# lRomul/sensorium

Measured on AMD Instinct MI355X. Metric: training clips/sec/GPU (DwiseNeuro fwd+bwd, B=32 T=32 36x64) at 1/2/4/8 GPUs, higher is better.
Workload: dtype bf16

## Files before the change

sensorium_amd/_lib.py:

```python
from __future__ import annotations

import ctypes as C
import os
from pathlib import Path

import torch

_HERE = Path(__file__).resolve().parent
DETERMINISTIC = os.environ.get("DWN_DETERMINISTIC", "0") == "1"
_LIB_NAME = "libdwiseneuro_hip_det.so" if DETERMINISTIC else "libdwiseneuro_hip.so"
LIB_PATH = Path(os.environ["DWN_LIB_PATH"]) if os.environ.get("DWN_LIB_PATH") else _HERE / "csrc" / _LIB_NAME

c_p = C.c_void_p
c_i = C.c_int
c_ll = C.c_longlong
c_f = C.c_float
c_d = C.c_double
c_sz = C.c_size_t

DWN_F32, DWN_BF16 = 0, 1
DWN_NREP = 32
LD_PLAIN, LD_PE, LD_BNACT, LD_AFFINE2, LD_DY3, LD_GATE, LD_CAT1 = 0, 1, 2, 3, 4, 5, 6
EPI_STORE, EPI_READOUT, EPI_DG, EPI_STORE_CAT, EPI_DH3 = 0, 1, 2, 3, 4
NN_AUTO, NN_XL128, NN_XL256, NN_TILE128, NN_KD = 0, 1, 2, 3, 4
# ... 248 lines not shown
    _fields_ = [("N", c_i), ("L", c_i), ("gh", c_i), ("gw", c_i), ("fit_baseline", c_i), ("pad_", c_i), ("params", c_p), ("maps", c_p),
                ("profile", c_p), ("separability", c_p)]


CORR_STAT_ROWS, CORR_TILE = 8, 16
CORR_MEAN, CORR_SUM = 0, 1
GABOR_GAUSSIAN, GABOR_NONE = 0, 1
BLUR_MAX_RADIUS, BLUR_TAPS_STRIDE, MOMENTS_CHUNK = 16, 33, 4096
MEI_STEP, MEI_PROJECT = 0, 1
MEI_CONTRAST_MAX, MEI_CONTRAST_FIXED = 0, 1
TRIAL_STATE_ROWS, TRIAL_SCORE_ROWS, TRIAL_SUMMARY, TRIAL_TILE = 17, 5, 8, 4
NOISE_BINARY, NOISE_SPARSE = 0, 1
STA_SUMMARY = 8
GAUSS_PARAMS, GAUSS_TABLE = 7, 16
PAIR_TOTAL, PAIR_SIGNAL, PAIR_NOISE = 0, 1, 2
PAIR_TILE, PAIR_KSTEP, PAIR_SUMMARY, PAIR_ROW_STATS = 64, 4, 8, 8
MIX_BOX, MIX_BLEND = 0, 1
VID_U8, VID_F32 = 0, 1

_OLD_STRUCTS = {
    "dwn_load_desc": LoadDesc, "dwn_gemm_nn_args": GemmNNArgs, "dwn_gemm_tn_args": GemmTNArgs,
    "dwn_dw_spatial_fwd_args": DwSpatialFwdArgs, "dwn_dw_spatial_bwd_args": DwSpatialBwdArgs,
    "dwn_dw_temporal_fwd_args": DwTemporalFwdArgs, "dwn_dw_temporal_bwd_args": DwTemporalBwdArgs,
    "dwn_bn": BN, "dwn_stem_args": StemArgs, "dwn_block_args": BlockArgs, "dwn_pool_args": PoolArgs,
    "dwn_cortex_args": CortexArgs, "dwn_readout_args": ReadoutArgs, "dwn_tensor_entry": TensorEntry,
    "dwn_clip_src": ClipSrc, "dwn_clip_desc": ClipDesc, "dwn_pw_bwd_args": PwBwdArgs,
    "dwn_dw_spatial_rc_fwd_args": DwSpatialRcFwdArgs,
}
_NEW_STRUCTS = {
    "dwn_stem_input_grad_args": StemInputGradArgs,
    "dwn_guarded_entry": GuardedEntry, "dwn_step_guard": StepGuard, "dwn_gaze_args": GazeArgs,
    "dwn_corr_args": CorrArgs, "dwn_gabor_args": GaborArgs, "dwn_modulator_args": ModulatorArgs,
    "dwn_blur3d_args": Blur3dArgs, "dwn_clip_moments_args": ClipMomentsArgs, "dwn_mei_update_args": MeiUpdateArgs,
    "dwn_trial_desc": TrialDesc, "dwn_trial_group": TrialGroup, "dwn_trial_score_args": TrialScoreArgs,
    "dwn_spatial_gain_args": SpatialGainArgs, "dwn_noise_args": NoiseArgs, "dwn_sta_args": StaArgs,
    "dwn_gauss2d_args": Gauss2dArgs, "dwn_gauss2d_profile_args": Gauss2dProfileArgs,
    "dwn_pair_seg": PairSeg, "dwn_pair_args": PairArgs, "dwn_pair_compare_args": PairCompareArgs,
}
_STRUCTS = {**_OLD_STRUCTS, **_NEW_STRUCTS}


class _new(tuple):
    def __new__(cls, restype, argtypes):
        return super().__new__(cls, (restype, argtypes))


_P = C.POINTER
SYMBOLS = {
    "dwn_abi_version": (c_i, []),
    "dwn_source_hash": (C.c_char_p, []),
    "dwn_sizeof": (c_i, [C.c_char_p]),
    "dwn_last_error": (C.c_char_p, []),
    "dwn_profile_enable": (c_i, [C.c_ulonglong, c_i]),
    "dwn_profile_collect": (c_i, [c_i, _P(c_d), _P(c_ll)]),
    "dwn_gemm_nn": (c_i, [_P(GemmNNArgs), c_i, c_i, c_p]),
    "dwn_gemm_tn": (c_i, [_P(GemmTNArgs), c_i, c_i, c_p]),
    "dwn_dw_spatial_fwd": (c_i, [_P(DwSpatialFwdArgs), c_i, c_i, c_p]),
    "dwn_dw_spatial_bwd": (c_i, [_P(DwSpatialBwdArgs), c_i, c_i, c_p]),
    "dwn_dw_spatial_bwd_rc_supported": (c_i, [_P(DwSpatialBwdArgs), c_i]),
    "dwn_dw_spatial_fwd_rc_supported": (c_i, [_P(DwSpatialFwdArgs), c_i]),
    "dwn_dw_temporal_fwd": (c_i, [_P(DwTemporalFwdArgs), c_i, c_i, c_p]),
    "dwn_dw_temporal_bwd": (c_i, [_P(DwTemporalBwdArgs), c_i, c_i, c_p]),
    "dwn_dw_temporal_wide_fwd": _new(c_i, [_P(DwTemporalFwdArgs), c_i, c_i, c_p]),
    "dwn_dw_temporal_wide_bwd": _new(c_i, [_P(DwTemporalBwdArgs), c_i, c_i, c_p]),
    "dwn_bn_finalize": (c_i, [c_p, c_i, c_d, _P(BN), c_i, c_i, c_f, c_f, c_i, c_p]),
    "dwn_bn_bwd_finalize": (c_i, [c_p, c_d, _P(BN), c_p, c_i, c_i, c_p]),
    "dwn_pack_weight": (c_i, [c_p, c_p, c_i, c_i, c_i, c_i, c_i, c_i, c_i, c_i, c_p]),
    "dwn_stem_workspace_bytes": (c_sz, [_P(StemArgs)]),
    "dwn_stem_forward": (c_i, [_P(StemArgs), c_i, c_p]),
    "dwn_stem_backward": (c_i, [_P(StemArgs), c_i, c_p]),
    "dwn_stem_input_grad": _new(c_i, [_P(StemInputGradArgs), c_i, c_p]),
    "dwn_stem_backward_input": _new(c_i, [_P(StemArgs), c_p, c_i, c_p]),
    "dwn_block_workspace_bytes": (c_sz, [_P(BlockArgs), c_i]),
    "dwn_block_forward": (c_i, [_P(BlockArgs), c_i, c_p]),
    "dwn_block_backward": (c_i, [_P(BlockArgs), c_i, c_p]),
    "dwn_block_forward_writes": (c_i, [_P(BlockArgs)]),
    "dwn_pool_forward": (c_i, [_P(PoolArgs), c_i, c_p]),
    "dwn_pool_backward": (c_i, [_P(PoolArgs), c_i, c_p]),
    "dwn_cortex_workspace_bytes": (c_sz, [_P(CortexArgs), c_i]),
    "dwn_cortex_forward": (c_i, [_P(CortexArgs), c_i, c_p]),
    "dwn_cortex_backward": (c_i, [_P(CortexArgs), c_i, c_p]),
    "dwn_readout_workspace_bytes": (c_sz, [_P(ReadoutArgs), c_i]),
    "dwn_readout_wt_bytes": (c_sz, [_P(ReadoutArgs)]),
    "dwn_readout_forward": (c_i, [_P(ReadoutArgs), c_i, c_p]),
    "dwn_readout_backward": (c_i, [_P(ReadoutArgs), c_i, c_p]),
    "dwn_poisson_loss_forward": (c_i, [c_p, c_p, c_p, c_ll, c_ll, c_f, c_p, c_i, c_p]),
    "dwn_poisson_loss_backward": (c_i, [c_p, c_p, c_p, c_p, c_ll, c_ll, c_f, c_p, c_i, c_p]),
    "dwn_f64_to_f32": (c_i, [c_p, c_p, c_i, c_i, c_p]),
    "dwn_adamw_ema_multi": (c_i, [c_p, c_i, c_i, c_d, c_d, c_d, c_d, c_d, c_ll, c_d, c_d, c_i, c_p]),
    "dwn_ema_lerp_multi": (c_i, [c_p, c_i, c_i, c_d, c_i, c_p]),
    "dwn_grad_guard_workspace_bytes": _new(c_sz, [c_i, c_i]),
    "dwn_grad_sumsq_multi": _new(c_i, [c_p, c_i, c_i, c_d, c_p, c_sz, c_p, c_i, c_p]),
    "dwn_step_guard_finalize": _new(c_i, [c_p, c_p, c_d, c_i, c_p, c_i, c_p, c_i, c_p]),
    "dwn_adamw_ema_multi_guarded": _new(c_i, [c_p, c_i, c_i, c_d, c_d, c_d, c_d, c_d, c_d, c_d, c_p, c_i, c_p]),
    "dwn_conv_pw_bn_stats_workspace_bytes": (c_sz, [c_i]),
    "dwn_conv_pw_bn_stats": (c_i, [c_p, c_ll, c_ll, c_p, c_i, c_i, _P(BN), c_f, c_f, c_p, c_p, c_sz, c_i, c_i, c_p]),
    "dwn_pw_bwd_fused_supported": (c_i, [c_i, c_ll, c_i, c_i]),
    "dwn_pw_backward_workspace_bytes": (c_sz, [c_i, c_i, c_i]),
    "dwn_pw_backward": (c_i, [_P(PwBwdArgs), c_i, c_i, c_p]),
    "dwn_dw_spatial_rc_blob_bytes": (c_sz, [c_i, c_i]),
    "dwn_dw_spatial_rc_prep": (c_i, [c_p, c_p, c_p, c_i, c_i, c_p, c_i, c_p]),
    "dwn_dw_spatial_rc_supported": (c_i, [c_i, c_i, c_i, c_i, c_i, c_i, c_i]),
    "dwn_dw_spatial_fwd_rc": (c_i, [_P(DwSpatialRcFwdArgs), c_i, c_p]),
    "dwn_assemble_inputs": (c_i, [c_p, c_i, c_i, c_i, c_i, c_i, c_i, c_f, c_p, c_i, c_p]),
    "dwn_assemble_targets": (c_i, [c_p, c_i, c_i, c_p, c_p, c_i, c_i, c_p, c_i, c_p]),
    "dwn_gaze_shift_forward": _new(c_i, [_P(GazeArgs), c_i, c_p]),
    "dwn_gaze_shift_backward": _new(c_i, [_P(GazeArgs), c_i, c_p]),
    "dwn_plane_mean": _new(c_i, [c_p, c_i, c_i, c_i, c_i, c_i, c_i, c_i, c_p, c_i, c_p]),
    "dwn_corr_ws_bytes": _new(c_sz, [_P(CorrArgs)]),
    "dwn_corr_moments": _new(c_i, [_P(CorrArgs), c_i, c_p]),
    "dwn_corr_loss_finalize": _new(c_i, [_P(CorrArgs), c_i, c_p]),
    "dwn_corr_loss_backward": _new(c_i, [_P(CorrArgs), c_i, c_p]),
    "dwn_gabor_workspace_bytes": _new(c_sz, [_P(GaborArgs)]),
    "dwn_gabor_forward": _new(c_i, [_P(GaborArgs), c_i, c_p]),
    "dwn_gabor_backward": _new(c_i, [_P(GaborArgs), c_i, c_p]),
    "dwn_modulator_ws_bytes": _new(c_sz, [_P(ModulatorArgs)]),
    "dwn_modulator_forward": _new(c_i, [_P(ModulatorArgs), c_i, c_p]),
    "dwn_modulator_backward": _new(c_i, [_P(ModulatorArgs), c_i, c_p]),
    "dwn_blur3d_ws_bytes": _new(c_sz, [_P(Blur3dArgs)]),
    "dwn_clip_moments_ws_bytes": _new(c_sz, [_P(ClipMomentsArgs)]),
    "dwn_blur3d": _new(c_i, [_P(Blur3dArgs), c_i, c_p]),
    "dwn_clip_moments": _new(c_i, [_P(ClipMomentsArgs), c_i, c_p]),
    "dwn_mei_update": _new(c_i, [_P(MeiUpdateArgs), c_i, c_p]),
    "dwn_trial_score_ws_bytes": _new(c_sz, [_P(TrialScoreArgs)]),
    "dwn_trial_moments": _new(c_i, [_P(TrialScoreArgs), c_i, c_p]),
    "dwn_trial_score_finalize": _new(c_i, [_P(TrialScoreArgs), c_i, c_p]),
    "dwn_spatial_gain_ws_bytes": _new(c_sz, [_P(SpatialGainArgs)]),
    "dwn_spatial_gain_forward": _new(c_i, [_P(SpatialGainArgs), c_i, c_p]),
    "dwn_spatial_gain_backward": _new(c_i, [_P(SpatialGainArgs), c_i, c_p]),
    "dwn_pair_ldz": _new(c_ll, [c_i]),
    "dwn_pair_state_bytes": _new(c_sz, [_P(PairArgs)]),
    "dwn_pair_ws_bytes": _new(c_sz, [_P(PairArgs)]),
    "dwn_pair_compare_ws_bytes": _new(c_sz, [_P(PairCompareArgs)]),
    "dwn_pair_stage": _new(c_i, [_P(PairArgs), c_i, c_p]),
    "dwn_pair_syrk": _new(c_i, [_P(PairArgs), c_i, c_p]),
    "dwn_pair_corr_finalize": _new(c_i, [_P(PairArgs), c_i, c_p]),
    "dwn_pair_compare": _new(c_i, [_P(PairCompareArgs), c_i, c_p]),
    "dwn_gauss2d_ws_bytes": _new(c_sz, [_P(Gauss2dArgs)]),
    "dwn_gauss2d_fit": _new(c_i, [_P(Gauss2dArgs), c_i, c_p]),
    "dwn_gauss2d_profile": _new(c_i, [_P(Gauss2dProfileArgs), c_i, c_p]),
    "dwn_noise_forward": _new(c_i, [_P(NoiseArgs), c_i, c_p]),
    "dwn_sta_state_bytes": _new(c_sz, [_P(StaArgs)]),
    "dwn_sta_ws_bytes": _new(c_sz, [_P(StaArgs)]),
    "dwn_sta_accumulate": _new(c_i, [_P(StaArgs), c_i, c_p]),
    "dwn_sta_finalize": _new(c_i, [_P(StaArgs), c_i, c_p]),
}


class DwnError(RuntimeError):
    pass


HASH_SRCS = ("dwn_api.hip", "dwn_gemm.hip", "dwn_gemm_nn_1.hip", "dwn_gemm_nn_2.hip", "dwn_gemm_nn_3.hip", "dwn_gemm_nn_4.hip", "dwn_gemm_nn_5.hip",
             "dwn_gemm_nn_6.hip", "dwn_gemm_tn.hip", "dwn_pw_bwd.hip", "dwn_gemm_xl.hip", "dwn_gemm_kd.hip", "dwn_dwconv.hip", "dwn_dwrc.hip",
             "dwn_dwbwd.hip", "dwn_dwfwd.hip", "dwn_elementwise.hip", "dwn_data.hip", "dwn_gaze.hip", "dwn_modulator.hip", "dwn_spatial.hip", "dwn_mei.hip", "dwn_rf_fit.hip", "dwn_pairwise.hip", "dwn_trial_score.hip", "dwn_rf.hip", "dwn_corr.hip", "dwn_stim.hip", "dwn_common.h", "dwn_internal.h",
             "dwn_kernels.h", "dwn_launch.h", "dwn_gemm_nn.h", "dwn_gain.h", "dwn_reduce.h",
             "../../include/dwn.h")


def source_hash() -> str:
    import hashlib
    h = hashlib.sha256()
    for name in HASH_SRCS:
        h.update((_HERE / "csrc" / name).read_bytes())
    return h.hexdigest()[:16]


def _load():
    if not LIB_PATH.exists():
        raise ImportError(
            f"{LIB_PATH} is missing: build it with `python -c 'import __graft_entry__ as g; g.build()'` "
            f"(or `make -C {LIB_PATH.parent}`).  sensorium_amd has no fallback path.")
    lib = C.CDLL(str(LIB_PATH), mode=getattr(os, "RTLD_NOW", 2))
    ab = bool(os.environ.get("DWN_LIB_PATH"))
    for name, proto in SYMBOLS.items():
        if ab and isinstance(proto, _new) and not hasattr(lib, name):
            continue
        restype, argtypes = proto
        fn = getattr(lib, name)
        fn.restype = restype
        fn.argtypes = argtypes
    if lib.dwn_abi_version() != 7 and not (ab and lib.dwn_abi_version() == 6):
        raise ImportError("libdwiseneuro_hip.so ABI version mismatch")
    built, have = lib.dwn_source_hash().decode(), source_hash()
    if built != have and not os.environ.get("DWN_LIB_PATH"):
        raise ImportError(f"{LIB_PATH.name} was built from other sources (binary {built}, tree {have}): rebuild it with "
                          f"`make -C {LIB_PATH.parent}` — binaries are not in git, so what runs must be what is committed")
    for cname, struct in _STRUCTS.items():
        n = lib.dwn_sizeof(cname.encode())
        if n != C.sizeof(struct) and not (ab and (0 < n < C.sizeof(struct) or cname in _NEW_STRUCTS)):
            raise ImportError(f"struct layout mismatch for {cname}: C {n} bytes vs ctypes {C.sizeof(struct)}")
    return lib


lib = _load()


def check(rc: int, what: str = ""):
    if rc != 0:
        msg = lib.dwn_last_error()
        raise DwnError(f"{what} failed (rc={rc}): {msg.decode() if msg else ''}")
```

sensorium_amd/csrc/dwn_api.hip:

```cpp
#include "dwn_internal.h"
#include "dwn_kernels.h"
#include <string.h>
#include <math.h>

static thread_local char g_err[512] = "";
#ifndef DWN_EVAL_CHAIN
#define DWN_EVAL_CHAIN 1
#endif

extern "C" size_t dwn_dw_spatial_rc_blob_bytes(int E, int Cin);
extern "C" int dwn_dw_spatial_rc_supported(int dtype, int Cin, int E, int ks, int stride, int Hin, int Win);
extern "C" int dwn_dw_spatial_rc_prep(const float* w_pw, const float* w_dws, const float* bn1_coef, int E, int Cin, void* blob,
                                      int device, void* stream);
extern "C" int dwn_dw_spatial_fwd_rc(const dwn_dw_spatial_rc_fwd_args* a, int device, void* stream);
bool dw_spatial_bwd_rc_supported(const DwSpatialBwd& a, int dtype);
bool dw_spatial_fwd_rc_walk_supported(const DwSpatialFwd& a, int dtype);

int dwn_set_error(int code, const char* msg) {
    snprintf(g_err, sizeof(g_err), "dwn error %d: %s", code, msg ? msg : "");
    return code;
}

#define TRY(x) do { int rc__ = (x); if (rc__ != 0) return rc__; } while (0)

// ... 45 lines not shown
        }
        if (range) g_roctx_pop();
    }
};
}
#define PROF(fam, call) do { ProfScope ps__((fam), s); TRY(call); } while (0)
#define HIP_TRY(x) do { hipError_t e__ = (x); if (e__ != hipSuccess) return dwn_set_error((int)e__, hipGetErrorString(e__)); } while (0)
#define ENTER(device) do { g_err[0] = 0; HIP_TRY(hipSetDevice(device)); } while (0)

namespace {

struct Carver {
    char* base; size_t off; size_t cap;
    explicit Carver(void* b, size_t c) : base((char*)b), off(0), cap(c) {}
    template <class U> U* take(size_t n) {
        off = (off + 255) & ~(size_t)255;
        U* p = base ? (U*)(base + off) : (U*)nullptr;
        off += n * sizeof(U);
        return p;
    }
    bool ok() const { return base == nullptr || off <= cap; }
};

inline size_t tsize(int dtype) { return dtype == DWN_BF16 ? 2 : 4; }
inline size_t nstat(int C) { return (size_t)DWN_NREP * 2 * C; }

LoadDesc ld_plain(const void* p, i64 ld) {
    LoadDesc d; memset(&d, 0, sizeof(d));
    d.p = p; d.ld = ld;
    return d;
}
LoadDesc ld_bnact(const void* p, i64 ld, const float* coef, int C, int act, const float* gate, int gate_ld,
                  int rows_per_sample) {
    LoadDesc d = ld_plain(p, ld);
    d.v1 = coef; d.v2 = coef + C; d.act = act; d.gate = gate; d.gate_ld = gate_ld;
    d.rows_per_sample = rows_per_sample > 0 ? rows_per_sample : 1;
    return d;
}
LoadDesc ld_affine2(const void* p, const void* q, i64 ld, const float* abc, int C) {
    LoadDesc d = ld_plain(p, ld);
    d.q = q; d.v1 = abc; d.v2 = abc + C; d.v3 = abc + 2 * C;
    return d;
}
LoadDesc ld_pe(const void* p, i64 ld, const float* pe_t, const float* pe_h, const float* pe_w, int T, int H, int W) {
    LoadDesc d = ld_plain(p, ld);
    d.pe_t = pe_t; d.pe_h = pe_h; d.pe_w = pe_w; d.pT = T; d.pH = H; d.pW = W; d.pe_ld = (int)ld;
    return d;
}
LoadDesc ld_ycoef(const void* y, i64 ld, const float* coef, int C) {
    LoadDesc d = ld_plain(y, ld);
    d.v1 = coef; d.v2 = coef + C; d.v3 = coef + 2 * C; d.v4 = coef + 3 * C;
    return d;
}

BnFinJob fin_job(const double* stats, int stat_c, double count, const dwn_bn& bn, int C) {
    BnFinJob j; memset(&j, 0, sizeof(j));
    j.stats = stats; j.stat_c = stat_c; j.count = count; j.gamma = bn.gamma; j.beta = bn.beta;
    j.running_mean = bn.running_mean; j.running_var = bn.running_var; j.nbt = bn.num_batches_tracked; j.coef = bn.coef; j.C = C;
    return j;
}
BnBwdJob bwd_job(const double* stats, double count, const dwn_bn& bn, float* abc, int C, bool frozen) {
    BnBwdJob j; memset(&j, 0, sizeof(j));
    j.stats = stats; j.count = count; j.coef = bn.coef; j.dgamma = bn.dgamma; j.dbeta = bn.dbeta; j.abc = abc; j.C = C;
    j.frozen = frozen ? 1 : 0;
    return j;
}

int bn_finalize(const double* stats, int stat_c, double count, const dwn_bn& bn, int C, int training, float momentum,
                float eps, hipStream_t s) {
    if (training) return k_bn_finalize_train(fin_job(stats, stat_c, count, bn, C), BnFinJob{}, momentum, eps, s);
    return k_bn_finalize_eval(bn.gamma, bn.beta, bn.running_mean, bn.running_var, eps, bn.coef, C, s);
}

GemmNN nn_base(const LoadDesc& a, int a_kind, const void* b, i64 ldb, void* c, i64 ldc, int M, int N, int K, int groups) {
    GemmNN g; memset(&g, 0, sizeof(g));
    g.a = a; g.a_kind = a_kind; g.b = b; g.ldb = ldb; g.c = c; g.ldc = ldc; g.M = M; g.N = N; g.K = K;
    g.groups = groups; g.epi = EPI_STORE;
    return g;
}
GemmTN tn_base(const LoadDesc& p, int pk, const LoadDesc& q, int qk, int M, int R, int Cc, float* dw, i64 lddw, int groups) {
    GemmTN g; memset(&g, 0, sizeof(g));
    g.p = p; g.p_kind = pk; g.q = q; g.q_kind = qk; g.M = M; g.R = R; g.Cc = Cc; g.dw = dw; g.lddw = lddw;
    g.groups = groups; g.nsplit = 0;
    return g;
}

struct BlockWs {
    void *wpw, *wpwl;
    float *wdws, *wdwt;
    double *st1, *st2, *st3, *st4, *stsc;
    long long* pooled;
    float *abc1, *abc2, *abc3, *abc4, *abcsc, *ident3;
    float *dgp, *dhp, *dps;
    void* bp; float* r3; float* gacc;
    float* tacc;
    void* wgated;
    void* rcblob;
    double* gram;
    float* pb;
    char* zero_beg; char* zero_end;
    size_t bytes;
};
#ifndef PWL_GATED_MIN_ROWS
#define PWL_GATED_MIN_ROWS 8192
#endif
static bool pwl_gated_weights(const dwn_block_args& a) {
    const int bk = a.dtype == DWN_BF16 ? 64 : 32;
    return ((a.T * a.Hout * a.Wout) % 128) == 0 && a.Cmid > bk && (a.dtype != DWN_BF16 || a.T * a.Hout * a.Wout >= PWL_GATED_MIN_ROWS);
}
static bool pwl_bwd_per_sample(const dwn_block_args& a) {
#ifdef DWN_DETERMINISTIC
    return true;
#endif
    if (a.pwl_bwd == 2) return false;
    if (a.pwl_bwd == 1) return true;
    const double pb = 4.0 * a.B * a.Cout * a.Cmid * sizeof(float);
    const double pass = (double)a.B * a.T * a.Hout * a.Wout * a.Cmid * tsize(a.dtype);
    return pb <= pass;
}
static bool block_y1_free(const dwn_block_args& a) {
    if (!a.training || a.dtype != DWN_BF16 || a.y1_mode == 1) return false;
    DwSpatialFwd f; memset(&f, 0, sizeof(f));
    f.planes = a.B * a.T; f.Hin = a.Hin; f.Win = a.Win; f.Hout = a.Hout; f.Wout = a.Wout; f.C = a.Cmid; f.stride = a.stride; f.ks = a.ks;
    f.in.ld = a.Cmid; f.a0_ld = a.Cin; f.Cin = a.Cin;
    if (!dw_spatial_fwd_rc_walk_supported(f, a.dtype)) return false;
    DwSpatialBwd d; memset(&d, 0, sizeof(d));
    d.planes = a.B * a.T; d.Hin = a.Hin; d.Win = a.Win; d.Hout = a.Hout; d.Wout = a.Wout; d.C = a.Cmid; d.stride = a.stride; d.ks = a.ks;
    d.dy.ld = a.Cmid; d.y1.ld = a.Cmid; d.a0_ld = a.Cin; d.Cin = a.Cin;
    if (!dw_spatial_bwd_rc_supported(d, a.dtype)) return false;
    return a.y1_mode == 2 || a.Cin == 64;
}
static bool block_fwd_rc(const dwn_block_args& a) {
    return !a.training && dwn_dw_spatial_rc_supported(a.dtype, a.Cin, a.Cmid, a.ks, a.stride, a.Hin, a.Win) != 0;
}
static size_t pw_fold_floats(int Cin) { return (size_t)Cin * Cin + Cin; }
BlockWs carve_block(const dwn_block_args& a, int backward, void* base, size_t cap) {
    BlockWs w; memset(&w, 0, sizeof(w));
    Carver c(base, cap);
    const size_t ts = tsize(a.dtype);
    w.wpw = c.take<char>((size_t)a.Cmid * a.Cin * ts);
    w.wpwl = c.take<char>((size_t)a.Cout * a.Cmid * ts);
    w.wdws = c.take<float>((size_t)a.ks * a.ks * a.Cmid);
    w.wdwt = c.take<float>((size_t)a.kt * a.Cmid);
    if (!backward && pwl_gated_weights(a)) w.wgated = c.take<char>((size_t)a.B * a.Cout * a.Cmid * ts);
    if (!backward && block_fwd_rc(a)) w.rcblob = c.take<char>(dwn_dw_spatial_rc_blob_bytes(a.Cmid, a.Cin));
    c.take<char>(0);
    size_t z0 = (c.off + 255) & ~(size_t)255;
    w.st1 = c.take<double>(nstat(a.Cmid));
    w.st2 = c.take<double>(nstat(a.Cmid));
    w.st3 = c.take<double>(nstat(a.Cmid));
    w.st4 = c.take<double>(nstat(a.Cout));
    w.stsc = c.take<double>(nstat(backward ? a.Cout : a.Cin));
    w.pooled = c.take<long long>((size_t)a.B * a.Cmid);
    if (!backward && block_y1_free(a)) w.gram = c.take<double>((size_t)(a.Cin + 8) * a.Cin);
    size_t z1 = c.off;
    if (backward) {
        w.abc1 = c.take<float>(3 * (size_t)a.Cmid);
        w.abc2 = c.take<float>(3 * (size_t)a.Cmid);
        w.abc3 = c.take<float>(3 * (size_t)a.Cmid);
        w.abc4 = c.take<float>(3 * (size_t)a.Cout);
        w.abcsc = c.take<float>(3 * (size_t)a.Cout);
        w.ident3 = c.take<float>(3 * (size_t)a.Cmid);
        w.dgp = c.take<float>((size_t)a.B * a.Cmid);
        w.dhp = c.take<float>((size_t)a.B * a.se_r);
        w.dps = c.take<float>((size_t)a.B * a.Cmid);
        w.bp = c.take<char>((size_t)a.Cin * (a.Cmid + a.Cin) * ts);
        w.gacc = c.take<float>(pw_fold_floats(a.Cin));
        w.r3 = w.gacc + (size_t)a.Cin * a.Cin;
        w.tacc = c.take<float>(pw_wgrad_tacc_floats(a.Cmid, a.Cin));
        if (pwl_bwd_per_sample(a)) w.pb = c.take<float>((size_t)a.B * a.Cout * a.Cmid);
    }
    w.bytes = c.off + 256;
    if (base) { w.zero_beg = (char*)base + z0; w.zero_end = (char*)base + z1; }
    return w;
}

static inline int f32_split_of(int policy, bool eval_forward) {
    return policy == DWN_F32_SPLIT3 ? 1 : policy == DWN_F32_NATIVE ? 0 : (eval_forward ? 1 : 0);
}

ResGeom geom_of(const dwn_block_args& a) {
    ResGeom gm;
    gm.BT = a.B * a.T; gm.T = a.T; gm.Hin = a.Hin; gm.Win = a.Win; gm.Hout = a.Hout; gm.Wout = a.Wout;
    gm.Cin = a.Cin; gm.Cout = a.Cout; gm.hsrc = a.hsrc; gm.wsrc = a.wsrc; gm.hinv = a.hinv; gm.winv = a.winv;
    return gm;
}

int check_block(const dwn_block_args& a) {
    if (a.Cin % 8 || a.Cmid % 8 || a.Cout % 8) return dwn_set_error(-2, "block: channel counts must be multiples of 8");
    if (a.ks != 3 && a.ks != 5 && a.ks != 7) return dwn_set_error(-4, "block: spatial_kernel must be 3, 5 or 7 (the built set)");
    if (a.kt != 3 && a.kt != 5 && a.kt != 7 && a.kt != 9) return dwn_set_error(-4, "block: temporal_kernel must be 3, 5, 7 or 9 (the built set)");
    if (a.Hout != (a.Hin - 1) / a.stride + 1 || a.Wout != (a.Win - 1) / a.stride + 1)
        return dwn_set_error(-2, "block: Hout/Wout inconsistent with stride");
    return 0;
}

}

extern "C" {

int dwn_abi_version(void) { return DWN_ABI_VERSION; }
int dwn_sizeof(const char* name) {
#define SZ(T) if (strcmp(name, #T) == 0) return (int)sizeof(T)
    SZ(dwn_load_desc); SZ(dwn_gemm_nn_args); SZ(dwn_gemm_tn_args); SZ(dwn_dw_spatial_fwd_args);
    SZ(dwn_dw_spatial_bwd_args); SZ(dwn_dw_temporal_fwd_args); SZ(dwn_dw_temporal_bwd_args); SZ(dwn_bn);
    SZ(dwn_stem_args); SZ(dwn_block_args); SZ(dwn_pool_args); SZ(dwn_cortex_args); SZ(dwn_readout_args);
    SZ(dwn_tensor_entry); SZ(dwn_clip_src); SZ(dwn_clip_desc); SZ(dwn_pw_bwd_args); SZ(dwn_dw_spatial_rc_fwd_args);
    SZ(dwn_stem_input_grad_args); SZ(dwn_guarded_entry); SZ(dwn_step_guard); SZ(dwn_gaze_args);
    SZ(dwn_corr_args); SZ(dwn_gabor_args); SZ(dwn_modulator_args); SZ(dwn_spatial_gain_args);
    SZ(dwn_blur3d_args); SZ(dwn_clip_moments_args); SZ(dwn_mei_update_args);
    SZ(dwn_trial_desc); SZ(dwn_trial_group); SZ(dwn_trial_score_args);
    SZ(dwn_noise_args); SZ(dwn_sta_args); SZ(dwn_gauss2d_args); SZ(dwn_gauss2d_profile_args);
    SZ(dwn_pair_seg); SZ(dwn_pair_args); SZ(dwn_pair_compare_args);
#undef SZ
    return -1;
}
const char* dwn_last_error(void) { return g_err; }

int dwn_profile_enable(unsigned long long family_mask, int device) {
    ENTER(device);
    for (int f = 0; f < DWN_FAM_COUNT; ++f) {
        ProfFam& p = g_prof[f];
        p.used = 0;
        if (((family_mask >> f) & 1ull) && p.beg.empty()) {
            p.beg.resize(PROF_POOL); p.end.resize(PROF_POOL);
            for (size_t i = 0; i < PROF_POOL; ++i) { HIP_TRY(hipEventCreate(&p.beg[i])); HIP_TRY(hipEventCreate(&p.end[i])); }
        }
    }
    if (family_mask & DWN_PROF_ROCTX) (void)roctx_resolve();
    g_prof_mask = family_mask;
    return 0;
}
int dwn_profile_collect(int family, double* total_ms, long long* launches) {
    if (family < 0 || family >= DWN_FAM_COUNT) return dwn_set_error(-2, "profile_collect: bad family");
    ProfFam& p = g_prof[family];
    double tot = 0;
    for (size_t i = 0; i < p.used; ++i) {
        HIP_TRY(hipEventSynchronize(p.end[i]));
        float ms = 0;
        HIP_TRY(hipEventElapsedTime(&ms, p.beg[i], p.end[i]));
        tot += ms;
    }
    *total_ms = tot; *launches = (long long)p.used;
    p.used = 0;
    return 0;
}

int dwn_gemm_nn(const dwn_gemm_nn_args* a, int dtype, int device, void* stream) {
    ENTER(device);
    return launch_gemm_nn(*a, dtype, (hipStream_t)stream);
}
int dwn_gemm_tn(const dwn_gemm_tn_args* a, int dtype, int device, void* stream) {
    ENTER(device);
    return launch_gemm_tn(*a, dtype, (hipStream_t)stream);
}
int dwn_dw_spatial_fwd(const dwn_dw_spatial_fwd_args* a, int dtype, int device, void* stream) {
    ENTER(device);
    return launch_dw_spatial_fwd(*a, dtype, (hipStream_t)stream);
}
int dwn_dw_spatial_bwd(const dwn_dw_spatial_bwd_args* a, int dtype, int device, void* stream) {
    ENTER(device);
    return launch_dw_spatial_bwd(*a, dtype, (hipStream_t)stream);
}
int dwn_dw_spatial_bwd_rc_supported(const dwn_dw_spatial_bwd_args* a, int dtype) { return dw_spatial_bwd_rc_supported(*a, dtype) ? 1 : 0; }
int dwn_dw_spatial_fwd_rc_supported(const dwn_dw_spatial_fwd_args* a, int dtype) { return dw_spatial_fwd_rc_walk_supported(*a, dtype) ? 1 : 0; }
int dwn_dw_temporal_fwd(const dwn_dw_temporal_fwd_args* a, int dtype, int device, void* stream) {
    ENTER(device);
    if (a->kt != 3 && a->kt != 5) return dwn_set_error(-4, "dw_temporal: only temporal_kernel 3 or 5 is built");
    return launch_dw_temporal_fwd(*a, dtype, (hipStream_t)stream);
}
int dwn_dw_temporal_bwd(const dwn_dw_temporal_bwd_args* a, int dtype, int device, void* stream) {
    ENTER(device);
    if (a->kt != 3 && a->kt != 5) return dwn_set_error(-4, "dw_temporal: only temporal_kernel 3 or 5 is built");
    return launch_dw_temporal_bwd(*a, dtype, (hipStream_t)stream);
}
int dwn_dw_temporal_wide_fwd(const dwn_dw_temporal_fwd_args* a, int dtype, int device, void* stream) {
    g_err[0] = 0;
    if (int rc = dw_temporal_wide_check(a->kt, a->C, LD_PLAIN)) return rc;
    ENTER(device);
    return launch_dw_temporal_wide_fwd(*a, dtype, (hipStream_t)stream);
}
int dwn_dw_temporal_wide_bwd(const dwn_dw_temporal_bwd_args* a, int dtype, int device, void* stream) {
    g_err[0] = 0;
    if (int rc = dw_temporal_wide_check(a->kt, a->C, a->dy_kind)) return rc;
    ENTER(device);
    return launch_dw_temporal_wide_bwd(*a, dtype, (hipStream_t)stream);
}
int dwn_bn_finalize(const double* stats, int stat_c, double count, const dwn_bn* bn, int C, int training,
                    float momentum, float eps, int device, void* stream) {
    ENTER(device);
    return bn_finalize(stats, stat_c, count, *bn, C, training, momentum, eps, (hipStream_t)stream);
}
int dwn_bn_bwd_finalize(const double* stats, double count, const dwn_bn* bn, float* abc, int C, int device,
                        void* stream) {
    ENTER(device);
    return k_bn_bwd_finalize(bwd_job(stats, count, *bn, abc, C, false), BnBwdJob{}, (hipStream_t)stream);
}
size_t dwn_conv_pw_bn_stats_workspace_bytes(int Cin) { return (size_t)(Cin + 8) * Cin * sizeof(double) + 256; }
int dwn_conv_pw_bn_stats(const void* a0, long long a0_ld, long long M, const float* w_pw, int E, int Cin, const dwn_bn* bn,
                         float momentum, float eps, double* sc_stats, void* ws, size_t ws_bytes, int dtype, int device, void* stream) {
    ENTER(device);
    hipStream_t s = (hipStream_t)stream;
    if (!a0 || !w_pw || !bn || !bn->coef || !ws) return dwn_set_error(-1, "conv_pw_bn_stats: null pointer");
    if (Cin % 8 || E <= 0 || M <= 0 || M >= (1ll << 31)) return dwn_set_error(-2, "conv_pw_bn_stats: Cin % 8 == 0, 0 < M < 2^31");
    if (ws_bytes < dwn_conv_pw_bn_stats_workspace_bytes(Cin)) return dwn_set_error(-6, "conv_pw_bn_stats: workspace too small");
    double* gram = reinterpret_cast<double*>(((size_t)ws + 255) & ~(size_t)255);
    TRY(k_zero(gram, (size_t)(Cin + 8) * Cin * sizeof(double), s));
    LoadDesc cat = ld_plain(a0, a0_ld);
    cat.cat_c1 = Cin; cat.cat_c2 = 0;
    GemmTN g = tn_base(cat, LD_CAT1, ld_plain(a0, a0_ld), LD_PLAIN, (int)M, Cin + 8, Cin, reinterpret_cast<float*>(gram), Cin, 1);
    g.dw_f64 = 1;
    TRY(launch_gemm_tn(g, dtype, s));
    return k_bn1_gram_finalize(gram, w_pw, E, Cin, (double)M, bn->gamma, bn->beta, bn->running_mean, bn->running_var,
                               bn->num_batches_tracked, momentum, eps, bn->coef, sc_stats, dtype, s);
}
int dwn_pack_weight(const float* src, void* dst, int groups, int R, int C, int transpose, int Rd, int Cd, int dtype,
                    int device, void* stream) {
    ENTER(device);
    return k_pack_weight(src, dst, groups, R, C, transpose, Rd, Cd, dtype, (hipStream_t)stream);
}

size_t dwn_stem_workspace_bytes(const dwn_stem_args* a) {
    return ((size_t)DWN_NREP * stem_moment_count() * sizeof(double) + 256 +
            (size_t)DWN_NREP * a->C0 * stem_acc_stride() * sizeof(double) + 1024);
}
int dwn_stem_forward(const dwn_stem_args* a, int device, void* stream) {
    ENTER(device);
    hipStream_t s = (hipStream_t)stream;
    if (a->C0 % 8) return dwn_set_error(-2, "stem: C0 must be a multiple of 8");
    if (a->pe_t && (i64)a->T * a->H * a->W != a->S) return dwn_set_error(-2, "stem: T*H*W != S");
    Carver c(a->ws, a->ws_bytes);
    double* mom = c.take<double>((size_t)DWN_NREP * stem_moment_count());
    if (!c.ok()) return dwn_set_error(-6, "stem: workspace too small");
    const i64 M = (i64)a->B * a->S;
    if (a->training == DWN_BN_TRAIN) {
        if (!a->xmom) return dwn_set_error(-1, "stem_forward: xmom buffer required in training mode");
        TRY(k_zero(mom, (size_t)DWN_NREP * stem_moment_count() * sizeof(double), s));
        TRY(k_stem_xmom(a->x, a->B, a->Cin, a->S, mom, s));
        TRY(k_stem_bn_finalize(mom, (double)M, a->w, a->bn.gamma, a->bn.beta, a->bn.running_mean, a->bn.running_var,
                               a->bn.num_batches_tracked, a->momentum, a->eps, a->bn.coef, a->xmom, a->C0, a->Cin, s));
    } else {
        TRY(bn_finalize(nullptr, a->C0, (double)M, a->bn, a->C0, 0, a->momentum, a->eps, s));
    }
    return k_stem_out(a->x, a->w, a->bn.coef, a->pe_t, a->pe_h, a->pe_w, a->T, a->H, a->W, a->B, a->Cin, a->S, a->C0, a->out,
                      a->dtype, s);
}
int dwn_stem_backward(const dwn_stem_args* a, int device, void* stream) {
    ENTER(device);
    hipStream_t s = (hipStream_t)stream;
    const bool frozen = a->training == DWN_BN_FROZEN;
    if (!frozen && !a->xmom) return dwn_set_error(-1, "stem_backward: xmom (saved by the forward) required");
    Carver c(a->ws, a->ws_bytes);
    double* mom = c.take<double>((size_t)DWN_NREP * stem_moment_count());
    double* acc = c.take<double>((size_t)DWN_NREP * a->C0 * stem_acc_stride());
    if (!c.ok()) return dwn_set_error(-6, "stem: workspace too small");
    const i64 M = (i64)a->B * a->S;
    if (frozen) {
        TRY(k_zero(mom, (size_t)((char*)(acc + (size_t)DWN_NREP * a->C0 * stem_acc_stride()) - (char*)mom), s));
        TRY(k_stem_bwd_acc(a->dout, a->x, mom, (double)M, a->B, a->Cin, a->S, a->C0, acc, a->dtype, s));
        return k_stem_bwd_finalize_frozen(acc, a->w, a->bn.coef, a->bn.dgamma, a->bn.dbeta, a->dw, a->C0, a->Cin, s);
    }
    TRY(k_zero(acc, (size_t)DWN_NREP * a->C0 * stem_acc_stride() * sizeof(double), s));
    TRY(k_stem_bwd_acc(a->dout, a->x, a->xmom, (double)M, a->B, a->Cin, a->S, a->C0, acc, a->dtype, s));
    return k_stem_bwd_finalize(acc, a->xmom, a->w, a->bn.coef, (double)M, a->bn.dgamma, a->bn.dbeta, a->dw, a->C0, a->Cin, s);
}

int dwn_stem_backward_input(const dwn_stem_args* a, float* dx, int device, void* stream) {
    g_err[0] = 0;
    if (!a || !dx) return dwn_set_error(-1, "stem_backward_input: null pointer (args, dx)");
    if (a->training != DWN_BN_TRAIN)
        return dwn_set_error(-7, "stem_backward_input: built for batch statistics (DWN_BN_TRAIN) only; the frozen-statistics input "
                                 "gradient is dwn_stem_backward + dwn_stem_input_grad");
    if (!a->x || !a->w || !a->bn.coef || !a->dout || !a->dw || !a->xmom || !a->ws)
        return dwn_set_error(-1, "stem_backward_input: null pointer (x, w, bn.coef, dout, dw, xmom, ws)");
    if (a->C0 <= 0 || a->C0 % 8 || a->Cin <= 0 || a->B <= 0 || a->S <= 0)
        return dwn_set_error(-2, "stem_backward_input: C0 must be a positive multiple of 8; B, Cin, S positive");
    if (a->dtype != DWN_F32 && a->dtype != DWN_BF16) return dwn_set_error(-2, "stem_backward_input: dtype");
    if (a->C0 > (a->dtype == DWN_BF16 ? 128 : 64) || a->Cin > 8)
        return dwn_set_error(-4, "stem_backward_input: more than 128 (bf16) / 64 (fp32) stem channels or 8 input channels not built");
    ENTER(device);
    hipStream_t s = (hipStream_t)stream;
    Carver c(a->ws, a->ws_bytes);
    double* mom = c.take<double>((size_t)DWN_NREP * stem_moment_count());
    double* acc = c.take<double>((size_t)DWN_NREP * a->C0 * stem_acc_stride());
    if (!c.ok()) return dwn_set_error(-6, "stem: workspace too small");
    float* qx = reinterpret_cast<float*>(mom);
    const i64 M = (i64)a->B * a->S;
    TRY(k_zero(acc, (size_t)DWN_NREP * a->C0 * stem_acc_stride() * sizeof(double), s));
    TRY(k_stem_bwd_acc(a->dout, a->x, a->xmom, (double)M, a->B, a->Cin, a->S, a->C0, acc, a->dtype, s));
    TRY(k_stem_bwd_finalize(acc, a->xmom, a->w, a->bn.coef, (double)M, a->bn.dgamma, a->bn.dbeta, a->dw, a->C0, a->Cin, s));
    TRY(k_stem_bwd_finalize_dx(acc, a->xmom, a->w, a->bn.coef, (double)M, qx, a->C0, a->Cin, s));
    return k_stem_input_grad_train(a->dout, a->w, a->bn.coef, a->x, qx, a->B, a->Cin, a->S, a->C0, dx, a->dtype, s);
}

int dwn_stem_input_grad(const dwn_stem_input_grad_args* a, int device, void* stream) {
    g_err[0] = 0;
    if (!a || !a->w || !a->coef || !a->dout || !a->dx) return dwn_set_error(-1, "stem_input_grad: null pointer");
    if (a->C0 <= 0 || a->C0 % 8 || a->Cin <= 0 || a->B <= 0 || a->S <= 0)
        return dwn_set_error(-2, "stem_input_grad: C0 must be a positive multiple of 8; B, Cin, S positive");
    if (a->dtype != DWN_F32 && a->dtype != DWN_BF16) return dwn_set_error(-2, "stem_input_grad: dtype");
    if (a->training != DWN_BN_FROZEN)
        return dwn_set_error(-7, "stem_input_grad: this entry is the frozen-statistics (DWN_BN_FROZEN) input gradient; through batch "
                                 "statistics (DWN_BN_TRAIN) it is dwn_stem_backward_input");
    ENTER(device);
    return k_stem_input_grad(a->dout, a->w, a->coef, a->B, a->Cin, a->S, a->C0, a->dx, a->dtype, (hipStream_t)stream);
}

size_t dwn_block_workspace_bytes(const dwn_block_args* a, int backward) {
    return carve_block(*a, backward, nullptr, 0).bytes;
}

int dwn_block_forward(const dwn_block_args* ap, int device, void* stream) {
    ENTER(device);
    const dwn_block_args& a = *ap;
    hipStream_t s = (hipStream_t)stream;
    TRY(check_block(a));
    BlockWs w = carve_block(a, 0, a.ws, a.ws_bytes);
    if (w.bytes > a.ws_bytes) return dwn_set_error(-6, "block_forward: workspace too small");
    const int dt = a.dtype, tr = a.training != DWN_BN_EVAL;
    const bool bs = a.training == DWN_BN_TRAIN;
    const i64 Min = (i64)a.B * a.T * a.Hin * a.Win, Mout = (i64)a.B * a.T * a.Hout * a.Wout;
    const int S_out = a.T * a.Hout * a.Wout;
    {
        PrepArgs pa;
        bool ok = pa.zero(w.zero_beg, ((size_t)(w.zero_end - w.zero_beg) + 15) & ~(size_t)15);
        ok = ok && pa.packw(a.w_pw, w.wpw, 1, a.Cmid, a.Cin, 0, a.Cmid, a.Cin);
        ok = ok && pa.packw(a.w_pwl, w.wpwl, 1, a.Cout, a.Cmid, 0, a.Cout, a.Cmid);
        ok = ok && pa.packdw(a.w_dws, w.wdws, a.Cmid, a.ks * a.ks);
        ok = ok && pa.packdw(a.w_dwt, w.wdwt, a.Cmid, a.kt);
        if (!bs) {
            ok = ok && pa.bneval(a.bn1, a.Cmid, a.eps) && pa.bneval(a.bn2, a.Cmid, a.eps) && pa.bneval(a.bn3, a.Cmid, a.eps);
            ok = ok && pa.bneval(a.bn4, a.Cout, a.eps) && pa.bneval(a.bnsc, a.Cout, a.eps);
        }
        if (!ok) return dwn_set_error(-2, "block_forward: workspace arena must be 16-byte aligned");
        TRY(k_prep(pa, dt, s));
    }

    const void* a0 = a.x;
    if (!a.x_has_pe) {
        if (!a.a0) return dwn_set_error(-2, "block_forward: a0 buffer required when x_has_pe == 0");
        TRY(k_ew_apply(ld_pe(a.x, a.Cin, a.pe_t, a.pe_h, a.pe_w, a.T, a.Hin, a.Win), LD_PE, a.a0, a.Cin, Min, a.Cin, dt, s));
        a0 = a.a0;
    }
    LoadDesc xin = ld_plain(a0, a.Cin);
    const bool identity_sc = a.stride == 1 && a.Hin == a.Hout && a.Win == a.Wout;
    const bool y1_free = tr && block_y1_free(a);
    bool eval_chain = false;
    if (DWN_EVAL_CHAIN && !tr && dt == DWN_BF16) {
        DwSpatialFwd f; memset(&f, 0, sizeof(f));
        f.planes = a.B * a.T; f.Hin = a.Hin; f.Win = a.Win; f.Hout = a.Hout; f.Wout = a.Wout; f.C = a.Cmid; f.stride = a.stride; f.ks = a.ks;
        f.in.ld = a.Cmid; f.a0_ld = a.Cin; f.Cin = a.Cin;
        eval_chain = dw_spatial_fwd_rc_walk_supported(f, dt);
    }
    if (eval_chain) {
        DwSpatialFwd d; memset(&d, 0, sizeof(d));
        d.in = ld_bnact(nullptr, a.Cmid, a.bn1.coef, a.Cmid, 1, nullptr, 0, 1);
        d.a0 = a0; d.a0_ld = a.Cin; d.w1 = w.wpw; d.Cin = a.Cin;
        d.w = w.wdws; d.out = a.y2; d.planes = a.B * a.T; d.Hin = a.Hin; d.Win = a.Win; d.Hout = a.Hout;
        d.Wout = a.Wout; d.C = a.Cmid; d.stride = a.stride; d.ks = a.ks; d.stats = nullptr;
        PROF(DWN_FAM_DWS_FWD, launch_dw_spatial_fwd(d, dt, s));
    } else if (y1_free) {
        LoadDesc cat = ld_plain(a0, a.Cin);
        cat.cat_c1 = a.Cin; cat.cat_c2 = 0;
        if (bs) {
        GemmTN g = tn_base(cat, LD_CAT1, ld_plain(a0, a.Cin), LD_PLAIN, (int)Min, a.Cin + 8, a.Cin, reinterpret_cast<float*>(w.gram), a.Cin, 1);
        g.dw_f64 = 1;
        PROF(DWN_FAM_PW_FWD, launch_gemm_tn(g, dt, s));
        PROF(DWN_FAM_PW_FWD, k_bn1_gram_finalize(w.gram, a.w_pw, a.Cmid, a.Cin, (double)Min, a.bn1.gamma, a.bn1.beta, a.bn1.running_mean,
                                                 a.bn1.running_var, a.bn1.num_batches_tracked, a.momentum, a.eps, a.bn1.coef,
                                                 identity_sc ? w.stsc : nullptr, dt, s));
        }
        DwSpatialFwd d; memset(&d, 0, sizeof(d));
        d.in = ld_bnact(nullptr, a.Cmid, a.bn1.coef, a.Cmid, 1, nullptr, 0, 1);
        d.a0 = a0; d.a0_ld = a.Cin; d.w1 = w.wpw; d.Cin = a.Cin;
        d.w = w.wdws; d.out = a.y2; d.planes = a.B * a.T; d.Hin = a.Hin; d.Win = a.Win; d.Hout = a.Hout;
        d.Wout = a.Wout; d.C = a.Cmid; d.stride = a.stride; d.ks = a.ks; d.stats = w.st2;
        PROF(DWN_FAM_DWS_FWD, launch_dw_spatial_fwd(d, dt, s));
    } else if (block_fwd_rc(a)) {
        TRY(dwn_dw_spatial_rc_prep(a.w_pw, w.wdws, a.bn1.coef, a.Cmid, a.Cin, w.rcblob, device, stream));
        dwn_dw_spatial_rc_fwd_args r; memset(&r, 0, sizeof(r));
        r.a0 = a0; r.a0_ld = a.Cin; r.blob = w.rcblob; r.out = a.y2; r.planes = a.B * a.T; r.Hin = a.Hin; r.Win = a.Win;
        r.Hout = a.Hout; r.Wout = a.Wout; r.Cin = a.Cin; r.E = a.Cmid; r.stride = a.stride; r.stats = nullptr;
        r.rows_band = 0; r.round_y1 = 1;
        PROF(DWN_FAM_DWS_FWD, dwn_dw_spatial_fwd_rc(&r, device, stream));
    } else {
    {
        GemmNN g = nn_base(xin, LD_PLAIN, w.wpw, a.Cin, a.y1, a.Cmid, (int)Min, a.Cmid, a.Cin, 1);
        g.f32_split = f32_split_of(a.f32_products, !tr);
        g.stats = tr ? w.st1 : nullptr; g.stat_nchan = a.Cmid;
        PROF(DWN_FAM_PW_FWD, launch_gemm_nn(g, dt, s));
    }
    if (bs) TRY(bn_finalize(w.st1, a.Cmid, (double)Min, a.bn1, a.Cmid, 1, a.momentum, a.eps, s));
    {
        DwSpatialFwd d; memset(&d, 0, sizeof(d));
        d.in = ld_bnact(a.y1, a.Cmid, a.bn1.coef, a.Cmid, 1, nullptr, 0, 1);
        d.w = w.wdws; d.out = a.y2; d.planes = a.B * a.T; d.Hin = a.Hin; d.Win = a.Win; d.Hout = a.Hout;
        d.Wout = a.Wout; d.C = a.Cmid; d.stride = a.stride; d.ks = a.ks; d.stats = tr ? w.st2 : nullptr;
        PROF(DWN_FAM_DWS_FWD, launch_dw_spatial_fwd(d, dt, s));
    }
    }
    if (bs) TRY(bn_finalize(w.st2, a.Cmid, (double)Mout, a.bn2, a.Cmid, 1, a.momentum, a.eps, s));
    const bool eval_z3 = !tr;
    {
        DwTemporalFwd d; memset(&d, 0, sizeof(d));
        d.in = ld_bnact(a.y2, a.Cmid, a.bn2.coef, a.Cmid, 1, nullptr, 0, 1);
        d.w = w.wdwt; d.out = a.y3; d.B = a.B; d.T = a.T; d.HW = a.Hout * a.Wout; d.C = a.Cmid; d.kt = a.kt;
        d.stats = tr ? w.st3 : nullptr;
        if (eval_z3) {
            d.out = a.z3; d.z_scale = a.bn3.coef; d.z_shift = a.bn3.coef + a.Cmid; d.pooled = w.pooled;
        }
        PROF(DWN_FAM_DWT_FWD, launch_dw_temporal_fwd(d, dt, s));
    }
    if (bs) TRY(bn_finalize(w.st3, a.Cmid, (double)Mout, a.bn3, a.Cmid, 1, a.momentum, a.eps, s));
    if (!eval_z3) {
        LoadDesc z3 = ld_bnact(a.y3, a.Cmid, a.bn3.coef, a.Cmid, 1, nullptr, 0, S_out);
        PROF(DWN_FAM_SE_POOL, k_se_pool(z3, a.B, a.Cmid, S_out, w.pooled, a.z3, dt, s));
    }
    int gate_folded = 0;
    TRY(k_se_mlp_fwd(w.pooled, 1.0f / (float)S_out, a.se_wr, a.se_br, a.se_we, a.se_be, a.B, a.Cmid, a.se_r,
                     a.se_pmean, a.se_hidpre, a.se_gate, pwl_gated_weights(a) ? a.w_pwl : nullptr, w.wgated, a.Cout, dt, &gate_folded, s));
    if (pwl_gated_weights(a)) {
        if (!gate_folded) TRY(k_gate_weights(a.w_pwl, a.se_gate, w.wgated, a.B, a.Cout, a.Cmid, dt, s));
        GemmNN g = nn_base(ld_plain(a.z3, a.Cmid), LD_PLAIN, w.wgated, a.Cmid, a.y4, a.Cout, (int)Mout, a.Cout, a.Cmid, 1);
        g.b_sample_stride = (i64)a.Cout * a.Cmid; g.b_rows_per_sample = S_out;
        g.stats = tr ? w.st4 : nullptr; g.stat_nchan = a.Cout; g.f32_split = f32_split_of(a.f32_products, !tr);
        PROF(DWN_FAM_PWL_FWD, launch_gemm_nn(g, dt, s));
    } else {
        LoadDesc u = ld_plain(a.z3, a.Cmid);
        u.gate = a.se_gate; u.gate_ld = a.Cmid; u.rows_per_sample = S_out;
        GemmNN g = nn_base(u, LD_GATE, w.wpwl, a.Cmid, a.y4, a.Cout, (int)Mout, a.Cout, a.Cmid, 1);
        g.stats = tr ? w.st4 : nullptr; g.stat_nchan = a.Cout; g.f32_split = f32_split_of(a.f32_products, !tr);
        PROF(DWN_FAM_PWL_FWD, launch_gemm_nn(g, dt, s));
    }
    ResGeom gm = geom_of(a);
    if (bs) {
        if (!(y1_free && identity_sc)) PROF(DWN_FAM_RESID_FWD, k_shortcut_stats(xin, gm, w.stsc, dt, s));
        TRY(k_bn_finalize_train(fin_job(w.st4, a.Cout, (double)Mout, a.bn4, a.Cout),
                                 fin_job(w.stsc, a.Cin, (double)Mout, a.bnsc, a.Cout), a.momentum, a.eps, s));
    }
    PROF(DWN_FAM_RESID_FWD, k_residual_fwd(xin, a.y4, a.bn4.coef, a.bnsc.coef, a.drop_scale, gm, a.out_pe_t, a.out_pe_h,
                                           a.out_pe_w, a.out, dt, s));
    return 0;
}

static int pw_backward(int dt, const void* dh1, const void* a0, const float* w_pw, const float* abc, int E, int Cin, i64 M,
                       void* bp, float* gacc, float* r3, float* tacc, void* da0, float* dw, const void* res,
                       const float* res_abc, int res_C, const ResGeom* rg, hipStream_t s) {
    const int res_n = res ? res_C / Cin : 0;
    const bool gathered = res && rg && rg->hinv;
    if (res && (!res_abc || res_C % Cin || res_n < 1 || res_n > 2))
        return dwn_set_error(-2, "pw_backward: the shortcut term needs res_abc and res_C in {Cin, 2 Cin}");
    if (res && !pw_bwd_fused_supported(dt, M, E, Cin))
        return dwn_set_error(-3, "pw_backward: the shortcut term is built into the one-pass kernel only (dwn_pw_bwd_fused_supported)");
    TRY(k_pw_bwd_prep(w_pw, abc, E, Cin, bp, gacc, r3, dt, (res && !gathered) ? res_abc : nullptr, res_C, s));
    if (pw_bwd_fused_supported(dt, M, E, Cin)) {
        PROF(DWN_FAM_PW_DGRAD, launch_pw_bwd_fused(dh1, a0, bp, r3, da0, tacc, M, E, Cin, dt, res, res_abc, res_n,
                                                   gathered ? rg->hinv : nullptr, gathered ? rg->winv : nullptr, gathered ? rg->Hin : 0,
                                                   gathered ? rg->Win : 0, gathered ? rg->Hout : 0, gathered ? rg->Wout : 0, s));
    } else {
        {
            GemmNN g = nn_base(ld_plain(dh1, E), LD_PLAIN, bp, (i64)E + Cin, da0, Cin, (int)M, Cin, E + Cin, 1);
            g.epi = EPI_STORE_CAT; g.a2 = a0; g.a2_ld = Cin; g.K1 = E; g.bias = r3;
            PROF(DWN_FAM_PW_DGRAD, launch_gemm_nn(g, dt, s));
        }
        {
            LoadDesc cat = ld_plain(dh1, E);
            cat.q = a0; cat.ld2 = Cin; cat.cat_c1 = E; cat.cat_c2 = Cin;
            GemmTN g = tn_base(cat, LD_CAT1, ld_plain(a0, Cin), LD_PLAIN, (int)M, E + Cin + 8, Cin, tacc, Cin, 1);
            PROF(DWN_FAM_PW_WGRAD, launch_gemm_tn(g, dt, s));
        }
    }
    return k_pw_wgrad_fold(tacc, abc, w_pw, E, Cin, dw, dt, s);
}

int dwn_block_backward(const dwn_block_args* ap, int device, void* stream) {
    const dwn_block_args& a = *ap;
    hipStream_t s = (hipStream_t)stream;
    g_err[0] = 0;
    TRY(check_block(a));
    if (a.training == DWN_BN_EVAL)
        return dwn_set_error(-7, "block_backward: only training-mode (batch-statistics) and frozen-statistics backward are built");
    ENTER(device);
    const bool frozen = a.training == DWN_BN_FROZEN;
    BlockWs w = carve_block(a, 1, a.ws, a.ws_bytes);
    if (w.bytes > a.ws_bytes) return dwn_set_error(-6, "block_backward: workspace too small");
    const int dt = a.dtype;
    const i64 Min = (i64)a.B * a.T * a.Hin * a.Win, Mout = (i64)a.B * a.T * a.Hout * a.Wout;
    const int S_out = a.T * a.Hout * a.Wout;
    float* dg = reinterpret_cast<float*>(w.pooled);
    const bool y1_free = block_y1_free(a);
    {
        PrepArgs pa;
        bool ok = pa.zero(w.zero_beg, ((size_t)(w.zero_end - w.zero_beg) + 15) & ~(size_t)15);
        ok = ok && pa.packw(a.w_pwl, w.wpwl, 1, a.Cout, a.Cmid, 1, a.Cmid, a.Cout);
        if (y1_free) ok = ok && pa.packw(a.w_pw, w.wpw, 1, a.Cmid, a.Cin, 0, a.Cmid, a.Cin);
        ok = ok && pa.packdw(a.w_dws, w.wdws, a.Cmid, a.ks * a.ks);
        ok = ok && pa.packdw(a.w_dwt, w.wdwt, a.Cmid, a.kt);
        ok = ok && pa.fill(w.ident3, 1.0f, a.Cmid);
        ok = ok && pa.fill(w.ident3 + a.Cmid, 0.0f, 2 * a.Cmid);
        ok = ok && pa.zero(a.dw_dws, (size_t)a.Cmid * a.ks * a.ks * sizeof(float));
        ok = ok && pa.zero(a.dw_dwt, (size_t)a.Cmid * a.kt * sizeof(float));
        ok = ok && pa.zero(a.dw_pwl, (size_t)a.Cout * a.Cmid * sizeof(float));
        if (w.pb) ok = ok && pa.zero(w.pb, (size_t)a.B * a.Cout * a.Cmid * sizeof(float));
        ok = ok && pa.zero(w.gacc, pw_fold_floats(a.Cin) * sizeof(float));
        ok = ok && pa.zero(w.tacc, pw_wgrad_tacc_floats(a.Cmid, a.Cin) * sizeof(float));
        if (!ok) return dwn_set_error(-2, "block_backward: workspace arena and dw_* buffers must be 16-byte aligned");
        TRY(k_prep(pa, dt, s));
    }

    LoadDesc xin = ld_plain(a.x_has_pe ? a.x : a.a0, a.Cin);
    ResGeom gm = geom_of(a);
    PROF(DWN_FAM_RESID_BWD, k_residual_bwd_reduce(xin, a.y4, a.dout, a.bn4.coef, a.bnsc.coef, a.drop_scale, gm, w.st4, w.stsc, dt, s));
    TRY(k_bn_bwd_finalize(bwd_job(w.st4, (double)Mout, a.bn4, w.abc4, a.Cout, frozen),
                          bwd_job(w.stsc, (double)Mout, a.bnsc, w.abcsc, a.Cout, frozen), s));
    PROF(DWN_FAM_RESID_BWD, k_residual_bwd_dy4(a.y4, a.dout, w.abc4, a.drop_scale, gm, a.dy4, dt, s));
    void* du = a.buf_a;
    if (w.pb) {
        {
            GemmTN g = tn_base(ld_plain(a.dy4, a.Cout), LD_PLAIN, ld_plain(a.z3, a.Cmid), LD_PLAIN, (int)Mout, a.Cout,
                               a.Cmid, w.pb, a.Cmid, 1);
            g.rows_per_sample = S_out; g.dw_sample_stride = (i64)a.Cout * a.Cmid;
            PROF(DWN_FAM_PWL_WGRAD, launch_gemm_tn(g, dt, s));
        }
        PROF(DWN_FAM_PWL_WGRAD, k_pwl_bwd_reduce(w.pb, a.se_gate, a.w_pwl, a.B, a.Cout, a.Cmid, a.dw_pwl, dg, s));
        TRY(k_se_mlp_bwd(dg, a.se_gate, a.se_hidpre, a.se_pmean, a.se_wr, a.se_we, a.B, a.Cmid, a.se_r,
                         1.0f / (float)S_out, w.dgp, w.dhp, w.dps, a.dse_wr, a.dse_br, a.dse_we, a.dse_be, s));
        GemmNN g = nn_base(ld_plain(a.dy4, a.Cout), LD_PLAIN, w.wpwl, a.Cout, du, a.Cmid, (int)Mout, a.Cmid, a.Cout, 1);
        g.epi = EPI_DH3; g.y3 = a.y3; g.ldy3 = a.Cmid; g.gate3 = a.se_gate; g.dps3 = w.dps; g.dg_ld = a.Cmid;
        g.coef3 = a.bn3.coef; g.coef3_ld = a.Cmid; g.rows_per_sample = S_out;
        g.stats = w.st3; g.stat_nchan = a.Cmid;
        PROF(DWN_FAM_PWL_DGRAD, launch_gemm_nn(g, dt, s));
    } else {
    {
        GemmNN g = nn_base(ld_plain(a.dy4, a.Cout), LD_PLAIN, w.wpwl, a.Cout, du, a.Cmid, (int)Mout, a.Cmid, a.Cout, 1);
        g.epi = EPI_DG; g.y3 = a.z3; g.ldy3 = a.Cmid; g.s3 = nullptr; g.t3 = nullptr; g.dg = dg;
        g.dg_ld = a.Cmid; g.rows_per_sample = S_out;
        PROF(DWN_FAM_PWL_DGRAD, launch_gemm_nn(g, dt, s));
    }
    {
        LoadDesc u = ld_plain(a.z3, a.Cmid);
        u.gate = a.se_gate; u.gate_ld = a.Cmid; u.rows_per_sample = S_out;
        GemmTN g = tn_base(ld_plain(a.dy4, a.Cout), LD_PLAIN, u, LD_GATE, (int)Mout, a.Cout, a.Cmid, a.dw_pwl, a.Cmid, 1);
        PROF(DWN_FAM_PWL_WGRAD, launch_gemm_tn(g, dt, s));
    }
    TRY(k_se_mlp_bwd(dg, a.se_gate, a.se_hidpre, a.se_pmean, a.se_wr, a.se_we, a.B, a.Cmid, a.se_r,
                     1.0f / (float)S_out, w.dgp, w.dhp, w.dps, a.dse_wr, a.dse_br, a.dse_we, a.dse_be, s));
    LoadDesc d3; memset(&d3, 0, sizeof(d3));
    d3.p = du; d3.q = a.y3; d3.ld = a.Cmid; d3.v1 = w.ident3; d3.v2 = w.ident3 + a.Cmid; d3.v3 = w.ident3 + 2 * a.Cmid;
    d3.v4 = a.bn3.coef; d3.v5 = a.bn3.coef + a.Cmid; d3.gate = a.se_gate; d3.gate2 = w.dps; d3.gate_ld = a.Cmid;
    d3.rows_per_sample = S_out;
    PROF(DWN_FAM_BN3_REDUCE, k_bn3_bwd_reduce(d3, a.bn3.coef, Mout, a.Cmid, w.st3, du, dt, s));
    }
    TRY(k_bn_bwd_finalize(bwd_job(w.st3, (double)Mout, a.bn3, w.abc3, a.Cmid, frozen), BnBwdJob{}, s));
    {
        DwTemporalBwd d; memset(&d, 0, sizeof(d));
        d.dy = ld_affine2(du, a.y3, a.Cmid, w.abc3, a.Cmid);
        d.dy_kind = LD_PLAIN;
        d.y2 = ld_ycoef(a.y2, a.Cmid, a.bn2.coef, a.Cmid);
        d.w = w.wdwt; d.dh2 = a.buf_b; d.dw = a.dw_dwt; d.B = a.B; d.T = a.T; d.HW = a.Hout * a.Wout; d.C = a.Cmid;
        d.kt = a.kt; d.stats = w.st2;
        PROF(DWN_FAM_DWT_BWD, launch_dw_temporal_bwd(d, dt, s));
    }
    TRY(k_bn_bwd_finalize(bwd_job(w.st2, (double)Mout, a.bn2, w.abc2, a.Cmid, frozen), BnBwdJob{}, s));
    void* dh1 = a.buf_a;
    {
        DwSpatialBwd d; memset(&d, 0, sizeof(d));
        d.dy = ld_affine2(a.buf_b, a.y2, a.Cmid, w.abc2, a.Cmid);
        d.y1 = ld_ycoef(y1_free ? nullptr : a.y1, a.Cmid, a.bn1.coef, a.Cmid);
        if (y1_free) { d.a0 = xin.p; d.a0_ld = a.Cin; d.w1 = w.wpw; d.Cin = a.Cin; }
        d.w = w.wdws; d.dh1 = dh1; d.dw = a.dw_dws; d.planes = a.B * a.T; d.Hin = a.Hin; d.Win = a.Win;
        d.Hout = a.Hout; d.Wout = a.Wout; d.C = a.Cmid; d.stride = a.stride; d.ks = a.ks; d.stats = w.st1;
        PROF(DWN_FAM_DWS_BWD, launch_dw_spatial_bwd(d, dt, s));
    }
    TRY(k_bn_bwd_finalize(bwd_job(w.st1, (double)Min, a.bn1, w.abc1, a.Cmid, frozen), BnBwdJob{}, s));
    const bool identity_sc = a.stride == 1 && a.Hin == a.Hout && a.Win == a.Wout;
    const bool dx_folded = a.Cout % a.Cin == 0 && a.Cout / a.Cin <= 2 && dwn_pw_bwd_fused_supported(dt, Min, a.Cmid, a.Cin) &&
                           (identity_sc || (gm.hinv && gm.winv && a.Hin + a.Win <= 512));
    TRY(pw_backward(dt, dh1, xin.p, a.w_pw, w.abc1, a.Cmid, a.Cin, Min, w.bp, w.gacc, w.r3, w.tacc, dx_folded ? a.dx : a.da0, a.dw_pw,
                    dx_folded ? a.dout : nullptr, w.abcsc, a.Cout, (dx_folded && !identity_sc) ? &gm : nullptr, s));
    if (dx_folded) return 0;
    PROF(DWN_FAM_RESID_BWD, k_residual_bwd_dx(xin, a.da0, a.dout, w.abcsc, gm, a.dx, dt, s));
    return 0;
}

int dwn_block_forward_writes(const dwn_block_args* ap) {
    const dwn_block_args& a = *ap;
    if (a.training) return block_y1_free(a) ? 2 : 3;
    if (block_fwd_rc(a)) return 0;
    if (DWN_EVAL_CHAIN && a.dtype == DWN_BF16) {
        DwSpatialFwd f; memset(&f, 0, sizeof(f));
        f.planes = a.B * a.T; f.Hin = a.Hin; f.Win = a.Win; f.Hout = a.Hout; f.Wout = a.Wout; f.C = a.Cmid; f.stride = a.stride; f.ks = a.ks;
        f.in.ld = a.Cmid; f.a0_ld = a.Cin; f.Cin = a.Cin;
        if (dw_spatial_fwd_rc_walk_supported(f, a.dtype)) return 0;
    }
    return 1;
}

int dwn_pool_forward(const dwn_pool_args* a, int device, void* stream) {
    ENTER(device);
    if (a->C % 8) return dwn_set_error(-2, "pool: C must be a multiple of 8");
    return k_pool_fwd(a->x, a->out, a->BT, a->HW, a->C, a->dtype, (hipStream_t)stream);
}
int dwn_pool_backward(const dwn_pool_args* a, int device, void* stream) {
    ENTER(device);
    if (a->C % 8) return dwn_set_error(-2, "pool: C must be a multiple of 8");
    return k_pool_bwd(a->dout, a->dx, a->BT, a->HW, a->C, a->dtype, (hipStream_t)stream);
}

namespace {
struct CortexWs { void* wp; double *st, *stsc; float *abc, *abcsc; void *dy, *dxmain; char *zb, *ze; size_t bytes; };
CortexWs carve_cortex(const dwn_cortex_args& a, int backward, void* base, size_t cap) {
    CortexWs w; memset(&w, 0, sizeof(w));
    Carver c(base, cap);
    const size_t ts = tsize(a.dtype);
    const i64 M = (i64)a.B * a.T;
    w.wp = c.take<char>((size_t)a.C * (a.Cin / a.groups) * ts);
    c.take<char>(0);
    size_t z0 = (c.off + 255) & ~(size_t)255;
    w.st = c.take<double>(nstat(a.C));
    w.stsc = c.take<double>(nstat(backward ? a.C : a.Cin));
    size_t z1 = c.off;
    if (backward) {
        w.abc = c.take<float>(3 * (size_t)a.C);
        w.abcsc = c.take<float>(3 * (size_t)a.C);
        w.dy = c.take<char>((size_t)M * a.C * ts);
        w.dxmain = c.take<char>((size_t)M * a.Cin * ts);
    }
    w.bytes = c.off + 256;
    if (base) { w.zb = (char*)base + z0; w.ze = (char*)base + z1; }
    return w;
}
}

size_t dwn_cortex_workspace_bytes(const dwn_cortex_args* a, int backward) {
    return carve_cortex(*a, backward, nullptr, 0).bytes;
}
int dwn_cortex_forward(const dwn_cortex_args* ap, int device, void* stream) {
    ENTER(device);
    const dwn_cortex_args& a = *ap;
    hipStream_t s = (hipStream_t)stream;
    if (a.Cin % (8 * a.groups) || a.C % (8 * a.groups)) return dwn_set_error(-2, "cortex: channels per group must be multiples of 8");
    CortexWs w = carve_cortex(a, 0, a.ws, a.ws_bytes);
    if (w.bytes > a.ws_bytes) return dwn_set_error(-6, "cortex_forward: workspace too small");
    const int M = a.B * a.T, Kg = a.Cin / a.groups, Ng = a.C / a.groups, dt = a.dtype, tr = a.training != DWN_BN_EVAL;
    const bool bs = a.training == DWN_BN_TRAIN;
    {
        PrepArgs pa;
        bool ok = pa.zero(w.zb, ((size_t)(w.ze - w.zb) + 15) & ~(size_t)15);
        ok = ok && pa.packw(a.w, w.wp, 1, a.C, Kg, 0, a.C, Kg);
        if (tr && !bs) ok = ok && pa.bneval(a.bn, a.C, a.eps) && pa.bneval(a.bnsc, a.C, a.eps);
        if (!ok) return dwn_set_error(-2, "cortex_forward: workspace arena must be 16-byte aligned");
        TRY(k_prep(pa, dt, s));
    }
    GemmNN g = nn_base(ld_plain(a.x, a.Cin), LD_PLAIN, w.wp, Kg, a.y, a.C, M, Ng, Kg, a.groups);
    g.f32_split = f32_split_of(a.f32_products, !tr);
    PROF(DWN_FAM_CORTEX_FWD, launch_gemm_nn(g, dt, s));
    if (bs) {
        TRY(k_cortex_stats(a.y, a.x, M, a.Cin, a.C, w.st, w.stsc, dt, s));
        TRY(k_bn_finalize_train(fin_job(w.st, a.C, (double)M, a.bn, a.C), fin_job(w.stsc, a.Cin, (double)M, a.bnsc, a.C),
                                 a.momentum, a.eps, s));
    } else if (!tr) {
        TRY(bn_finalize(w.st, a.C, (double)M, a.bn, a.C, 0, a.momentum, a.eps, s));
        TRY(bn_finalize(w.stsc, a.Cin, (double)M, a.bnsc, a.C, 0, a.momentum, a.eps, s));
    }
    return k_cortex_residual_fwd(a.y, a.x, a.bn.coef, a.bnsc.coef, a.drop_scale, M, a.T, a.Cin, a.C, a.groups, a.out,
                                 dt, s);
}
int dwn_cortex_backward(const dwn_cortex_args* ap, int device, void* stream) {
    const dwn_cortex_args& a = *ap;
    hipStream_t s = (hipStream_t)stream;
    g_err[0] = 0;
    if (a.training == DWN_BN_EVAL) return dwn_set_error(-7, "cortex_backward: only training-mode and frozen-statistics backward are built");
    ENTER(device);
    const bool frozen = a.training == DWN_BN_FROZEN;
    CortexWs w = carve_cortex(a, 1, a.ws, a.ws_bytes);
    if (w.bytes > a.ws_bytes) return dwn_set_error(-6, "cortex_backward: workspace too small");
    const int M = a.B * a.T, Kg = a.Cin / a.groups, Ng = a.C / a.groups, dt = a.dtype;
    {
        PrepArgs pa;
        bool ok = pa.zero(w.zb, ((size_t)(w.ze - w.zb) + 15) & ~(size_t)15);
        ok = ok && pa.packw(a.w, w.wp, a.groups, Ng, Kg, 1, Kg, Ng);
        ok = ok && pa.zero(a.dw, (size_t)a.C * Kg * sizeof(float));
        if (!ok) return dwn_set_error(-2, "cortex_backward: workspace arena and dw must be 16-byte aligned (C * Cin / groups a multiple of 4)");
        TRY(k_prep(pa, dt, s));
    }
    TRY(k_cortex_bwd_reduce(a.y, a.x, a.dout, a.dout_mask, a.dout_mask_ld, a.bn.coef, a.bnsc.coef, a.drop_scale, M, a.T,
                            a.Cin, a.C, a.groups, w.st, w.stsc, dt, s));
    TRY(k_bn_bwd_finalize(bwd_job(w.st, (double)M, a.bn, w.abc, a.C, frozen), bwd_job(w.stsc, (double)M, a.bnsc, w.abcsc, a.C, frozen), s));
    TRY(k_cortex_bwd_dy(a.y, a.dout, a.dout_mask, a.dout_mask_ld, a.bn.coef, w.abc, a.drop_scale, M, a.T, a.C, a.groups,
                        w.dy, dt, s));
    {
        GemmNN g = nn_base(ld_plain(w.dy, a.C), LD_PLAIN, w.wp, Ng, w.dxmain, a.Cin, M, Kg, Ng, a.groups);
        PROF(DWN_FAM_CORTEX_BWD, launch_gemm_nn(g, dt, s));
    }
    {
        GemmTN g = tn_base(ld_plain(w.dy, a.C), LD_PLAIN, ld_plain(a.x, a.Cin), LD_PLAIN, M, Ng, Kg, a.dw, Kg, a.groups);
        PROF(DWN_FAM_CORTEX_BWD, launch_gemm_tn(g, dt, s));
    }
    return k_cortex_bwd_dx(w.dxmain, a.x, a.dout, a.dout_mask, a.dout_mask_ld, w.abcsc, M, a.T, a.Cin, a.C, a.dx, dt, s);
}

namespace {
struct ReadoutWs { void* wp; void* dz; void* xd; double* dbp; size_t bytes; int Npad, Rg, Rp, ldp, ldt; };
ReadoutWs carve_readout(const dwn_readout_args& a, int backward, void* base, size_t cap) {
    ReadoutWs w; memset(&w, 0, sizeof(w));
    Carver c(base, cap);
    const size_t ts = tsize(a.dtype);
    const i64 M = (i64)a.B * a.T;
    w.Npad = (a.n_out + a.groups - 1) / a.groups * a.groups;
    w.Rg = w.Npad / a.groups;
    w.Rp = (w.Rg + 63) / 64 * 64;
    const int Kg = a.Cin / a.groups;
    w.ldp = Kg; w.ldt = w.Rp;
    w.wp = c.take<char>(backward ? (a.wt ? 0 : (size_t)a.groups * Kg * w.ldt * ts) : (size_t)w.Npad * w.ldp * ts);
    if (backward) w.dz = c.take<char>((size_t)M * a.groups * w.Rp * ts);
    if (a.drop_mask) w.xd = c.take<char>((size_t)M * a.Cin * ts);
    if (backward && a.beta_dev) w.dbp = c.take<double>(k_readout_dbeta_parts(a.B, w.Rp, a.groups));
    w.bytes = c.off + 256;
    return w;
}
}

size_t dwn_readout_workspace_bytes(const dwn_readout_args* a, int backward) {
    return carve_readout(*a, backward, nullptr, 0).bytes;
}
size_t dwn_readout_wt_bytes(const dwn_readout_args* a) {
    ReadoutWs w = carve_readout(*a, 0, nullptr, 0);
    return (size_t)a->groups * (a->Cin / a->groups) * w.ldt * tsize(a->dtype);
}
int dwn_readout_forward(const dwn_readout_args* ap, int device, void* stream) {
    ENTER(device);
    const dwn_readout_args& a = *ap;
    hipStream_t s = (hipStream_t)stream;
    if (a.Cin % (8 * a.groups)) return dwn_set_error(-2, "readout: in-channels per group must be a multiple of 8");
    ReadoutWs w = carve_readout(a, 0, a.ws, a.ws_bytes);
// ... 614 lines not shown
```

sensorium_amd/csrc/dwn_elementwise.hip:

```cpp
#include "dwn_internal.h"
#include "dwn_kernels.h"
#include "dwn_launch.h"

#define NCV 8
#define DISPATCH_T(dtype, CALL_BF, CALL_F) do { if ((dtype) == DWN_BF16) { CALL_BF; } else { CALL_F; } } while (0)

#define SLICE_SETUP(Cval)                                   \
    constexpr int KC = TT<T>::KC;                           \
    const int tid = threadIdx.x;                            \
    const int cv = tid % NCV, pl = tid / NCV;               \
    const int c0 = blockIdx.y * NCV * KC;                   \
    const int chan = c0 + cv * KC;                          \
    const bool chan_ok = chan < (Cval);                     \
    (void)pl; (void)chan_ok;

template <int KC>
__device__ __forceinline__ void slice_stats_flush(float* lstat, const float* s0, const float* s1, int cv,
                                                 int c0, int C, double* stats, int rep) {
    static_assert(NCV == 8, "wave pre-reduction below assumes 8 channel vectors per slice");
    const int tid = threadIdx.x;
    DET_WAVES_BEGIN
#pragma unroll
    for (int i = 0; i < KC; ++i) {
        float a = s0[i], b = s1[i];
#pragma unroll
        for (int o = 8; o < 64; o <<= 1) { a += __shfl_xor(a, o); b += __shfl_xor(b, o); }
        if ((tid & 63) < NCV) {
            atomicAdd(&lstat[cv * KC + i], a);
            atomicAdd(&lstat[NCV * KC + cv * KC + i], b);
        }
    }
    DET_WAVES_END
    __syncthreads();
    DET_ENTER();
    if (tid < 2 * NCV * KC) {
        int which = tid / (NCV * KC), c = c0 + tid % (NCV * KC);
        if (c < C) stat_add(stats, rep, C, which, c, lstat[tid]);
    }
}

template <typename K>
static dim3 resident_slice_grid(K kernel, i64 rows, int C, int KC, int max_bpc = 1 << 20) {
    int slices = (C + NCV * KC - 1) / (NCV * KC);
    int bpc = resident_bpc(kernel, 256, 0, 4);
    if (bpc > max_bpc) bpc = max_bpc;
    return dim3((unsigned)resident_grid_x(bpc, slices, (rows + 31) / 32), (unsigned)slices);
}

static inline dim3 slice_grid(i64 rows, int C, int KC, int cap = 2048) {
    int slices = (C + NCV * KC - 1) / (NCV * KC);
    i64 bx = (rows + 31) / 32;
    int capx = (cap + slices - 1) / slices;
    if (bx > capx) bx = capx;
    if (bx < 1) bx = 1;
    return dim3((unsigned)bx, (unsigned)slices);
}

static inline dim3 fat_slice_grid(i64 rows, int C, int KC) {
    int slices = (C + NCV * KC - 1) / (NCV * KC);
    i64 bx = 256 / slices;
    i64 need = (rows + (1024 / NCV) - 1) / (1024 / NCV);
    if (bx > need) bx = need;
    if (bx < 1) bx = 1;
    return dim3((unsigned)bx, (unsigned)slices);
}

static_assert(DWN_NREP == 32, "replica reduce below assumes 32 replicas");
__device__ __forceinline__ void rep_reduce(const double* stats, int stat_c, int sc, int r, bool ok, double& s, double& ss) {
    s = ok ? stats[((i64)r * 2 + 0) * stat_c + sc] : 0.0;
    ss = ok ? stats[((i64)r * 2 + 1) * stat_c + sc] : 0.0;
#pragma unroll
    for (int o = 16; o > 0; o >>= 1) { s += __shfl_xor(s, o); ss += __shfl_xor(ss, o); }
}

__device__ __forceinline__ void bn_finalize_train_body(const int blk, const double* stats, int stat_c, double count,
                                                       const float* gamma, const float* beta, float* running_mean,
                                                       float* running_var, long long* nbt, float momentum, float eps,
                                                       float* coef, int C) {
    const int r = threadIdx.x & 31;
    const int c = blk * 8 + (threadIdx.x >> 5);
    if (c == 0 && r == 0 && nbt) *nbt += 1;
    const bool ok = c < C;
    const int sc = ok ? c % stat_c : 0;
    double s, ss;
    rep_reduce(stats, stat_c, sc, r, ok, s, ss);
    if (!ok || r != 0) return;
    double mean = s / count;
    double var = ss / count - mean * mean;
    if (var < 0) var = 0;
    float invstd = (float)(1.0 / sqrt(var + (double)eps));
    float scale = gamma[c] * invstd;
    coef[c] = scale;
    coef[C + c] = beta[c] - (float)mean * scale;
    coef[2 * C + c] = (float)mean;
    coef[3 * C + c] = invstd;
    if (running_mean) {
        double unbiased = count > 1 ? var * count / (count - 1) : var;
        running_mean[c] = (1.f - momentum) * running_mean[c] + momentum * (float)mean;
        running_var[c] = (1.f - momentum) * running_var[c] + momentum * (float)unbiased;
    }
}
__global__ __launch_bounds__(256) void bn_finalize_train_kernel(BnFinJob j0, BnFinJob j1, float momentum, float eps) {
    const bool first = (int)blockIdx.x < j0.nblocks;
    const BnFinJob& j = first ? j0 : j1;
    bn_finalize_train_body(first ? blockIdx.x : blockIdx.x - j0.nblocks, j.stats, j.stat_c, j.count, j.gamma, j.beta,
                           j.running_mean, j.running_var, j.nbt, momentum, eps, j.coef, j.C);
}

__global__ void bn_finalize_eval_kernel(const float* gamma, const float* beta, const float* running_mean,
                                        const float* running_var, float eps, float* coef, int C) {
    int c = blockIdx.x * blockDim.x + threadIdx.x;
    if (c >= C) return;
    float invstd = 1.0f / sqrtf(running_var[c] + eps);
    float scale = gamma[c] * invstd;
    coef[c] = scale;
    coef[C + c] = beta[c] - running_mean[c] * scale;
    coef[2 * C + c] = running_mean[c];
    coef[3 * C + c] = invstd;
}

__device__ __forceinline__ void bn_bwd_finalize_body(const int blk, const double* stats, double count, const float* coef,
                                                     float* dgamma, float* dbeta, float* abc, int C, const bool frozen) {
    const int r = threadIdx.x & 31;
    const int c = blk * 8 + (threadIdx.x >> 5);
    const bool ok = c < C;
    double s1, s2;
    rep_reduce(stats, C, ok ? c : 0, r, ok, s1, s2);
    if (!ok || r != 0) return;
    float scale = coef[c], mean = coef[2 * C + c], invstd = coef[3 * C + c];
    if (dgamma) dgamma[c] = (float)s2;
    if (dbeta) dbeta[c] = (float)s1;
    double m1 = s1 / count, m2 = s2 / count;
    abc[c] = scale;
    abc[C + c] = frozen ? 0.f : (float)(-(double)scale * invstd * m2);
    abc[2 * C + c] = frozen ? 0.f : (float)((double)scale * (-m1 + (double)mean * invstd * m2));
}
__global__ __launch_bounds__(256) void bn_bwd_finalize_kernel(BnBwdJob j0, BnBwdJob j1) {
    const bool first = (int)blockIdx.x < j0.nblocks;
    const BnBwdJob& j = first ? j0 : j1;
    bn_bwd_finalize_body(first ? blockIdx.x : blockIdx.x - j0.nblocks, j.stats, j.count, j.coef, j.dgamma, j.dbeta, j.abc, j.C,
                         j.frozen != 0);
}

int k_bn_finalize_train(BnFinJob j0, BnFinJob j1, float momentum, float eps, hipStream_t s) {
    j0.nblocks = (j0.C + 7) / 8; j1.nblocks = (j1.C + 7) / 8;
    hipLaunchKernelGGL(bn_finalize_train_kernel, dim3(j0.nblocks + j1.nblocks), dim3(256), 0, s, j0, j1, momentum, eps);
    DWN_CHECK_LAUNCH();
    return 0;
}
int k_bn_bwd_finalize(BnBwdJob j0, BnBwdJob j1, hipStream_t s) {
    j0.nblocks = (j0.C + 7) / 8; j1.nblocks = (j1.C + 7) / 8;
    hipLaunchKernelGGL(bn_bwd_finalize_kernel, dim3(j0.nblocks + j1.nblocks), dim3(256), 0, s, j0, j1);
    DWN_CHECK_LAUNCH();
    return 0;
}
int k_bn_finalize_eval(const float* gamma, const float* beta, const float* rm, const float* rv, float eps,
                       float* coef, int C, hipStream_t s) {
    hipLaunchKernelGGL(bn_finalize_eval_kernel, dim3((C + 255) / 256), dim3(256), 0, s, gamma, beta, rm, rv, eps,
                       coef, C);
    DWN_CHECK_LAUNCH();
    return 0;
}

template <typename T>
__global__ __launch_bounds__(256) void bn1_gram_finalize_kernel(const double* __restrict__ gram, const float* __restrict__ w1,
                                                                int E, int Cin, double count, const float* gamma, const float* beta,
                                                                float* running_mean, float* running_var, long long* nbt,
                                                                float momentum, float eps, float* coef, double* sc_stats) {
    __shared__ float lw[4][512];
    const int lane = threadIdx.x & 63, wv = threadIdx.x >> 6;
    const int e = blockIdx.x * 4 + wv;
    if (blockIdx.x == 0 && threadIdx.x == 0 && nbt) *nbt += 1;
    if (sc_stats && blockIdx.x == 0) {
        for (int c = threadIdx.x; c < Cin; c += 256) {
            sc_stats[c] = gram[(i64)Cin * Cin + c];
            sc_stats[Cin + c] = gram[(i64)c * Cin + c];
        }
    }
    if (e >= E) return;
    for (int j = lane; j < Cin; j += 64) lw[wv][j] = round_t<T>(w1[(i64)e * Cin + j]);
    __builtin_amdgcn_wave_barrier();
    const double inv_n = 1.0 / count;
    double quad = 0.0, lin = 0.0;
    for (int i = lane; i < Cin; i += 64) {
        const double* grow = gram + (i64)i * Cin;
        double r = 0.0;
        for (int j = 0; j < Cin; j += 2) {
            const double2 g2 = *reinterpret_cast<const double2*>(grow + j);
            r += g2.x * (double)lw[wv][j] + g2.y * (double)lw[wv][j + 1];
        }
        quad += (double)lw[wv][i] * r;
        lin += (double)lw[wv][i] * gram[(i64)Cin * Cin + i];
    }
#pragma unroll
    for (int o = 32; o > 0; o >>= 1) { quad += __shfl_xor(quad, o); lin += __shfl_xor(lin, o); }
    if (lane != 0) return;
    const double mean = lin * inv_n;
    double var = quad * inv_n - mean * mean;
    if (var < 0) var = 0;
    const float invstd = (float)(1.0 / sqrt(var + (double)eps));
    const float scale = gamma[e] * invstd;
    coef[e] = scale;
    coef[E + e] = beta[e] - (float)mean * scale;
    coef[2 * E + e] = (float)mean;
    coef[3 * E + e] = invstd;
    if (running_mean) {
        const double unbiased = count > 1 ? var * count / (count - 1) : var;
        running_mean[e] = (1.f - momentum) * running_mean[e] + momentum * (float)mean;
        running_var[e] = (1.f - momentum) * running_var[e] + momentum * (float)unbiased;
    }
}
int k_bn1_gram_finalize(const double* gram, const float* w1, int E, int Cin, double count, const float* gamma, const float* beta,
                        float* rm, float* rv, long long* nbt, float momentum, float eps, float* coef, double* sc_stats, int dtype,
                        hipStream_t s) {
    if (Cin > 512 || Cin % 4) return dwn_set_error(-2, "bn1_gram_finalize: Cin must be a multiple of 4, at most 512");
    if (dtype == DWN_BF16)
        hipLaunchKernelGGL(bn1_gram_finalize_kernel<bf16_t>, dim3((E + 3) / 4), dim3(256), 0, s, gram, w1, E, Cin, count, gamma, beta,
                           rm, rv, nbt, momentum, eps, coef, sc_stats);
    else
        hipLaunchKernelGGL(bn1_gram_finalize_kernel<float>, dim3((E + 3) / 4), dim3(256), 0, s, gram, w1, E, Cin, count, gamma, beta,
                           rm, rv, nbt, momentum, eps, coef, sc_stats);
    DWN_CHECK_LAUNCH();
    return 0;
}

template <typename T, int KIND>
__global__ __launch_bounds__(256) void ew_apply_kernel(LoadDesc d, T* out, i64 ldo, i64 rows, int C) {
    SLICE_SETUP(C)
    if (!chan_ok) return;
    for (i64 row = (i64)blockIdx.x * 32 + pl; row < rows; row += (i64)gridDim.x * 32) {
        float v[KC];
        load_op<KIND, T>(d, row, chan, v);
        st_vec<T>(out + row * ldo + chan, v);
    }
}

template <typename T>
static int ew_apply_t(const LoadDesc& d, int kind, void* out, i64 ldo, i64 rows, int C, hipStream_t s) {
    dim3 grid = slice_grid(rows, C, TT<T>::KC);
    T* o = reinterpret_cast<T*>(out);
    switch (kind) {
        case LD_PLAIN: hipLaunchKernelGGL((ew_apply_kernel<T, LD_PLAIN>), grid, dim3(256), 0, s, d, o, ldo, rows, C); break;
        case LD_PE: hipLaunchKernelGGL((ew_apply_kernel<T, LD_PE>), grid, dim3(256), 0, s, d, o, ldo, rows, C); break;
        case LD_BNACT: hipLaunchKernelGGL((ew_apply_kernel<T, LD_BNACT>), grid, dim3(256), 0, s, d, o, ldo, rows, C); break;
        case LD_AFFINE2: hipLaunchKernelGGL((ew_apply_kernel<T, LD_AFFINE2>), grid, dim3(256), 0, s, d, o, ldo, rows, C); break;
        case LD_DY3: hipLaunchKernelGGL((ew_apply_kernel<T, LD_DY3>), grid, dim3(256), 0, s, d, o, ldo, rows, C); break;
        case LD_GATE: hipLaunchKernelGGL((ew_apply_kernel<T, LD_GATE>), grid, dim3(256), 0, s, d, o, ldo, rows, C); break;
        default: return dwn_set_error(-3, "ew_apply: bad loader kind");
    }
    DWN_CHECK_LAUNCH();
    return 0;
}
int k_ew_apply(const LoadDesc& d, int kind, void* out, i64 ldo, i64 rows, int C, int dtype, hipStream_t s) {
    return dtype == DWN_BF16 ? ew_apply_t<bf16_t>(d, kind, out, ldo, rows, C, s)
                             : ew_apply_t<float>(d, kind, out, ldo, rows, C, s);
}

constexpr int STEM_MAXCIN = 8;
constexpr int STEM_NM = STEM_MAXCIN + STEM_MAXCIN * STEM_MAXCIN;

__global__ __launch_bounds__(256) void stem_xmom_kernel(const float* x, int B, int Cin, i64 S, double* mom) {
    __shared__ double lsum[STEM_NM];
    const int tid = threadIdx.x;
    if (tid < STEM_NM) lsum[tid] = 0.0;
    __syncthreads();
    float sx[STEM_MAXCIN], xx[STEM_MAXCIN][STEM_MAXCIN];
#pragma unroll
    for (int a_ = 0; a_ < STEM_MAXCIN; ++a_) {
        sx[a_] = 0.f;
#pragma unroll
        for (int b_ = 0; b_ < STEM_MAXCIN; ++b_) xx[a_][b_] = 0.f;
    }
    const i64 rows = (i64)B * S;
    for (i64 row = (i64)blockIdx.x * 256 + tid; row < rows; row += (i64)gridDim.x * 256) {
        const i64 b = row / S, sp = row - b * S;
        float xv[STEM_MAXCIN];
#pragma unroll
        for (int c = 0; c < STEM_MAXCIN; ++c) xv[c] = c < Cin ? x[(b * Cin + c) * S + sp] : 0.f;
#pragma unroll
        for (int a_ = 0; a_ < STEM_MAXCIN; ++a_) {
            sx[a_] += xv[a_];
#pragma unroll
            for (int b_ = a_; b_ < STEM_MAXCIN; ++b_) xx[a_][b_] = fmaf(xv[a_], xv[b_], xx[a_][b_]);
        }
    }
    DET_WAVES_BEGIN
#pragma unroll
    for (int a_ = 0; a_ < STEM_MAXCIN; ++a_) {
        if (a_ >= Cin) break;
        double v = (double)sx[a_];
#pragma unroll
        for (int o = 32; o > 0; o >>= 1) v += __shfl_xor(v, o);
        if ((tid & 63) == 0) atomicAdd(&lsum[a_], v);
#pragma unroll
        for (int b_ = a_; b_ < STEM_MAXCIN; ++b_) {
            if (b_ >= Cin) break;
            double q = (double)xx[a_][b_];
#pragma unroll
            for (int o = 32; o > 0; o >>= 1) q += __shfl_xor(q, o);
            if ((tid & 63) == 0) atomicAdd(&lsum[STEM_MAXCIN + a_ * STEM_MAXCIN + b_], q);
        }
    }
    DET_WAVES_END
    __syncthreads();
    DET_ENTER();
    if (tid < STEM_NM) {
        const double v = lsum[tid];
        if (v != 0.0) atomicAdd(mom + (i64)(blockIdx.x % DWN_NREP) * STEM_NM + tid, v);
    }
    DET_EXIT();
}

__global__ __launch_bounds__(256) void stem_bn_finalize_kernel(const double* mom, double count, const float* w, const float* gamma,
                                                               const float* beta, float* running_mean, float* running_var,
                                                               long long* nbt, float momentum, float eps, float* coef,
                                                               double* xmom, int C0, int Cin) {
    __shared__ double lm[STEM_NM];
    const int tid = threadIdx.x;
    if (tid < STEM_NM) {
        double v = 0.0;
        for (int r = 0; r < DWN_NREP; ++r) v += mom[(i64)r * STEM_NM + tid];
        lm[tid] = v;
    }
    __syncthreads();
    if (tid < STEM_NM) {
        const int a_ = tid < STEM_MAXCIN ? 0 : (tid - STEM_MAXCIN) / STEM_MAXCIN, b_ = tid < STEM_MAXCIN ? 0 : (tid - STEM_MAXCIN) % STEM_MAXCIN;
        double v = lm[tid];
        if (tid >= STEM_MAXCIN && b_ < a_) v = lm[STEM_MAXCIN + b_ * STEM_MAXCIN + a_];
        xmom[tid] = v;
    }
    if (tid == 0 && nbt) *nbt += 1;
    for (int c = tid; c < C0; c += blockDim.x) {
        double mean = 0.0, var = 0.0;
        for (int a_ = 0; a_ < Cin; ++a_) mean += (double)w[c * Cin + a_] * (lm[a_] / count);
        for (int a_ = 0; a_ < Cin; ++a_)
            for (int b_ = 0; b_ < Cin; ++b_) {
                const double sxx = a_ <= b_ ? lm[STEM_MAXCIN + a_ * STEM_MAXCIN + b_] : lm[STEM_MAXCIN + b_ * STEM_MAXCIN + a_];
                const double cov = sxx / count - (lm[a_] / count) * (lm[b_] / count);
                var += (double)w[c * Cin + a_] * (double)w[c * Cin + b_] * cov;
            }
        if (var < 0) var = 0;
        const float invstd = (float)(1.0 / sqrt(var + (double)eps));
        const float scale = gamma[c] * invstd;
        coef[c] = scale;
        coef[C0 + c] = beta[c] - (float)mean * scale;
        coef[2 * C0 + c] = (float)mean;
        coef[3 * C0 + c] = invstd;
        if (running_mean) {
            const double unbiased = count > 1 ? var * count / (count - 1) : var;
            running_mean[c] = (1.f - momentum) * running_mean[c] + momentum * (float)mean;
            running_var[c] = (1.f - momentum) * running_var[c] + momentum * (float)unbiased;
        }
    }
}

template <typename T, int CINT>
__global__ __launch_bounds__(256) void stem_out_kernel(const float* x, const float* w, const float* coef, const float* pe_t,
                                                       const float* pe_h, const float* pe_w, int Tn, int H, int W, int B,
                                                       int Cin, i64 S, int C0, T* out) {
    SLICE_SETUP(C0)
    constexpr int STEM_MAXCIN = CINT;
    const int chs_ = chan_ok ? chan : 0;
    float wr[STEM_MAXCIN][KC], sc[KC], sh[KC];
#pragma unroll
    for (int c = 0; c < STEM_MAXCIN; ++c)
#pragma unroll
        for (int i = 0; i < KC; ++i) wr[c][i] = (c < Cin && chan_ok) ? w[(chan + i) * Cin + c] : 0.f;
// ... 925 lines not shown
    }
#pragma unroll
    for (int q = 0; q < RPW; ++q) {
        const float t = wave_sum(acc[q]);
        const int r = wave + 4 * q;
        if (lane == 0 && r < R) {
            const float h = t + br[r];
            if (part == 0) hid_pre[(i64)b * R + r] = h;
            hid[r] = siluf_(h);
        }
    }
    __syncthreads();
    const int per = (C + split - 1) / split;
    const int c_end = (part + 1) * per < C ? (part + 1) * per : C;
    for (int c = part * per + tid; c < c_end; c += 256) {
        float a = be[c];
        const float* wrow = we + (i64)c * R;
#pragma unroll 1
        for (int r0 = 0; r0 < RP; r0 += 16) {
            if (r0 >= R) break;
            float wv[16];
            if ((R & 3) == 0) {
                const float4* w4 = reinterpret_cast<const float4*>(wrow);
                const int nq = R >> 2;
#pragma unroll
                for (int q = 0; q < 4; ++q) {
                    const int qi = (r0 >> 2) + q;
                    const float4 t = w4[qi < nq ? qi : nq - 1];
                    wv[4 * q] = t.x; wv[4 * q + 1] = t.y; wv[4 * q + 2] = t.z; wv[4 * q + 3] = t.w;
                }
            } else {
#pragma unroll
                for (int r = 0; r < 16; ++r) wv[r] = wrow[r0 + r < R ? r0 + r : R - 1];
            }
#pragma unroll
            for (int r = 0; r < 16; ++r) a = fmaf(wv[r], r0 + r < R ? hid[r0 + r] : 0.f, a);
        }
        const float gv = sigmoidf_(a);
        gate[(i64)b * C + c] = gv;
        if (w2 && c - part * per < 256) gl[c - part * per] = gv;
    }
    if (w2) {
        __syncthreads();
        const int c0 = part * per, nc = c_end - c0;
        if (nc > 0) {
            const int tot = N2 * nc;
            for (int i = tid; i < tot; i += 256) {
                const int n = i / nc, cc = i - n * nc;
                const float v = w2[(i64)n * C + c0 + cc] * gl[cc];
                const i64 o = ((i64)b * N2 + n) * C + c0 + cc;
                if (wg_bf16) reinterpret_cast<bf16_t*>(wg)[o] = f2bf(v);
                else reinterpret_cast<float*>(wg)[o] = v;
            }
        }
    }
}

template <int N, int LIVE, int D> struct WaveFold {
    static __device__ __forceinline__ void run(float (&v)[N], int lane) {
        if constexpr (D > 0) {
            if constexpr (LIVE > D) {
                constexpr int H = LIVE / 2;
                const bool up = (lane & D) != 0;
#pragma unroll
                for (int i = 0; i < H; ++i) {
                    const float send = up ? v[i] : v[i + H];
                    const float keep = up ? v[i + H] : v[i];
                    v[i] = keep + __shfl_xor(send, D);
                }
                WaveFold<N, H, D / 2>::run(v, lane);
            } else {
#pragma unroll
                for (int i = 0; i < LIVE; ++i) v[i] += __shfl_xor(v[i], D);
                WaveFold<N, LIVE, D / 2>::run(v, lane);
            }
        }
    }
};
template <int N>
__device__ __forceinline__ float wave_fold(float (&v)[N], int lane) {
    WaveFold<N, N, 32>::run(v, lane);
    return v[0];
}

template <int RP, int VW>
__global__ __launch_bounds__(256) void se_mlp_bwd_fold_kernel(const float* dg, const float* gate, const float* hid_pre,
                                                              const float* wr, const float* we, int C, int R,
                                                              float inv_s, float* dgp_out, float* dhp_out, float* dps) {
    __shared__ float part4[4][RP];
    __shared__ float dhp[RP];
    const int b = blockIdx.x, tid = threadIdx.x, lane = tid & 63, wave = tid >> 6;
    const int split = gridDim.y, part = blockIdx.y;
    float acc[RP];
#pragma unroll
    for (int r = 0; r < RP; ++r) acc[r] = 0.f;
    for (int c = tid; c < C; c += 256) {
        const float g = gate[(i64)b * C + c];
        const float v = dg[(i64)b * C + c] * g * (1.f - g);
        if (part == 0) dgp_out[(i64)b * C + c] = v;
        const float* wrow = we + (i64)c * R;
        if constexpr (VW == 4) {
            const float4* w4 = reinterpret_cast<const float4*>(wrow);
            const int nq = R >> 2;
            float4 t[RP / 4];
#pragma unroll
            for (int q = 0; q < RP / 4; ++q) t[q] = w4[q < nq ? q : nq - 1];
#pragma unroll
            for (int q = 0; q < RP / 4; ++q) {
                acc[4 * q] = fmaf(t[q].x, v, acc[4 * q]); acc[4 * q + 1] = fmaf(t[q].y, v, acc[4 * q + 1]);
                acc[4 * q + 2] = fmaf(t[q].z, v, acc[4 * q + 2]); acc[4 * q + 3] = fmaf(t[q].w, v, acc[4 * q + 3]);
            }
        } else {
            const float2* w2 = reinterpret_cast<const float2*>(wrow);
            const int nq = R >> 1;
            float2 t[RP / 2];
#pragma unroll
            for (int q = 0; q < RP / 2; ++q) t[q] = w2[q < nq ? q : nq - 1];
#pragma unroll
            for (int q = 0; q < RP / 2; ++q) {
                acc[2 * q] = fmaf(t[q].x, v, acc[2 * q]); acc[2 * q + 1] = fmaf(t[q].y, v, acc[2 * q + 1]);
            }
        }
    }
    const float tot = wave_fold<RP>(acc, lane);
    if (lane < RP) part4[wave][lane] = tot;
    __syncthreads();
    if (tid < RP) {
        const float sum = (part4[0][tid] + part4[1][tid]) + (part4[2][tid] + part4[3][tid]);
        float v = 0.f;
        if (tid < R) {
            v = sum * silu_gradf_(hid_pre[(i64)b * R + tid]);
            if (part == 0) dhp_out[(i64)b * R + tid] = v;
        }
        dhp[tid] = v;
    }
    __syncthreads();
    const int per = (C + split - 1) / split;
    const int c_end = (part + 1) * per < C ? (part + 1) * per : C;
    for (int c = part * per + tid; c < c_end; c += 256) {
        float a = 0.f;
#pragma unroll 1
        for (int r0 = 0; r0 < RP; r0 += 16) {
            if (r0 >= R) break;
            float wv[16];
#pragma unroll
            for (int r = 0; r < 16; ++r) wv[r] = wr[(i64)(r0 + r < R ? r0 + r : R - 1) * C + c];
#pragma unroll
            for (int r = 0; r < 16; ++r) a = fmaf(wv[r], r0 + r < R ? dhp[r0 + r] : 0.f, a);
        }
        dps[(i64)b * C + c] = a * inv_s;
    }
}

__global__ __launch_bounds__(256) void se_mlp_wgrad_kernel(const float* dgp, const float* dhp, const float* pmean,
                                                           const float* hid_pre, int B, int C, int R, float* dwr,
                                                           float* dbr, float* dwe, float* dbe) {
    const int c = blockIdx.x * 256 + threadIdx.x;
    const int r = blockIdx.y;
    if (c < C) {
        float a = 0.f, a2 = 0.f, sb = 0.f;
#pragma unroll 8
        for (int b = 0; b < B; ++b) {
            float g = dgp[(i64)b * C + c];
            a = fmaf(g, siluf_(hid_pre[(i64)b * R + r]), a);
            a2 = fmaf(dhp[(i64)b * R + r], pmean[(i64)b * C + c], a2);
            sb += g;
        }
        dwe[(i64)c * R + r] = a;
        dwr[(i64)r * C + c] = a2;
        if (r == 0) dbe[c] = sb;
    }
    if (blockIdx.x == 0 && threadIdx.x == 0) {
        float sb = 0.f;
        for (int b = 0; b < B; ++b) sb += dhp[(i64)b * R + r];
        dbr[r] = sb;
    }
}

int k_se_mlp_fwd(const long long* pooled_sum, float inv_s, const float* wr, const float* br, const float* we,
                 const float* be, int B, int C, int R, float* pmean, float* hid_pre, float* gate, const float* w2, void* wg, int N2,
                 int dtype, int* folded, hipStream_t s) {
    if (folded) *folded = 0;
    if ((C & 3) == 0 && R <= SE_RT && !(((size_t)pooled_sum | (size_t)wr | (size_t)pmean) & 15)) {
        const bool fold = w2 && wg && (C + 7) / 8 <= 256;
        const float* w2f = fold ? w2 : nullptr;
        const int bf = dtype == DWN_BF16 ? 1 : 0;
        if (R <= 16)
            hipLaunchKernelGGL(se_mlp_fwd_rows_kernel<16>, dim3(B, 8), dim3(256), 0, s, pooled_sum, inv_s, wr, br, we, be, C, R,
                               pmean, hid_pre, gate, w2f, wg, N2, bf);
        else if (R <= 32)
            hipLaunchKernelGGL(se_mlp_fwd_rows_kernel<32>, dim3(B, 8), dim3(256), 0, s, pooled_sum, inv_s, wr, br, we, be, C, R,
                               pmean, hid_pre, gate, w2f, wg, N2, bf);
        else
            hipLaunchKernelGGL(se_mlp_fwd_rows_kernel<SE_RT>, dim3(B, 8), dim3(256), 0, s, pooled_sum, inv_s, wr, br, we, be, C,
                               R, pmean, hid_pre, gate, w2f, wg, N2, bf);
        if (folded && fold) *folded = 1;
    } else {
        hipLaunchKernelGGL(se_mlp_fwd_kernel, dim3(B, 8), dim3(256), (C + R) * sizeof(float), s, pooled_sum, inv_s, wr, br,
                           we, be, C, R, pmean, hid_pre, gate);
    }
    DWN_CHECK_LAUNCH();
    return 0;
}
int k_se_mlp_bwd(const float* dg, const float* gate, const float* hid_pre, const float* pmean, const float* wr,
                 const float* we, int B, int C, int R, float inv_s, float* dgp, float* dhp, float* dps, float* dwr,
                 float* dbr, float* dwe, float* dbe, hipStream_t s) {
    if ((R & 1) == 0 && R <= SE_RT && !((size_t)we & 15)) {
#define SE_BWD_FOLD(RP_) do { \
        if ((R & 3) == 0) hipLaunchKernelGGL((se_mlp_bwd_fold_kernel<RP_, 4>), dim3(B, 8), dim3(256), 0, s, dg, gate, hid_pre, wr, we, C, R, inv_s, dgp, dhp, dps); \
        else hipLaunchKernelGGL((se_mlp_bwd_fold_kernel<RP_, 2>), dim3(B, 8), dim3(256), 0, s, dg, gate, hid_pre, wr, we, C, R, inv_s, dgp, dhp, dps); } while (0)
        if (R <= 16) SE_BWD_FOLD(16);
        else if (R <= 32) SE_BWD_FOLD(32);
        else SE_BWD_FOLD(SE_RT);
#undef SE_BWD_FOLD
    } else {
        hipLaunchKernelGGL(se_mlp_bwd_kernel, dim3(B, 8), dim3(256), (C + R) * sizeof(float), s, dg, gate, hid_pre, wr, we,
                           C, R, inv_s, dgp, dhp, dps);
    }
    DWN_CHECK_LAUNCH();
    hipLaunchKernelGGL(se_mlp_wgrad_kernel, dim3((C + 255) / 256, R), dim3(256), 0, s, dgp, dhp, pmean, hid_pre, B, C, R,
                       dwr, dbr, dwe, dbe);
    DWN_CHECK_LAUNCH();
    return 0;
}

template <typename T>
__global__ __launch_bounds__(256) void bn3_bwd_reduce_kernel(LoadDesc d, const float* coef3, i64 rows, int C,
                                                             double* stats, T* dh_out) {
    SLICE_SETUP(C)
    __shared__ float lstat[2 * NCV * KC];
    if (tid < 2 * NCV * KC) lstat[tid] = 0.f;
    __syncthreads();
    float s0[KC], s1[KC];
#pragma unroll
    for (int i = 0; i < KC; ++i) { s0[i] = 0.f; s1[i] = 0.f; }
    if (chan_ok) {
        float m3[KC], i3[KC];
        ld_coef<KC>(coef3 + 2 * C + chan, m3);
        ld_coef<KC>(coef3 + 3 * C + chan, i3);
        const T* yp = reinterpret_cast<const T*>(d.q);
        const T* pp = reinterpret_cast<const T*>(d.p);
        float sc[KC], sh[KC], g[KC], g2[KC];
        ld_coef<KC>(d.v4 + chan, sc);
        ld_coef<KC>(d.v5 + chan, sh);
        int gb = -1;
        const i64 stride = (i64)gridDim.x * 32;
        for (i64 row0 = (i64)blockIdx.x * 32 + pl; row0 < rows; row0 += 2 * stride) {
            uint4 rp[2], ry[2];
#pragma unroll
            for (int u = 0; u < 2; ++u) {
                i64 row = row0 + u * stride;
                if (row >= rows) row = row0;
                rp[u] = *reinterpret_cast<const uint4*>(pp + row * d.ld + chan);
                ry[u] = *reinterpret_cast<const uint4*>(yp + row * d.ld + chan);
            }
#pragma unroll
            for (int u = 0; u < 2; ++u) {
                i64 row = row0 + u * stride;
                if (row >= rows) break;
                int b = (int)((unsigned)row / (unsigned)d.rows_per_sample);
                if (b != gb) {
                    gb = b;
                    ld_coef<KC>(d.gate + (i64)b * d.gate_ld + chan, g);
                    ld_coef<KC>(d.gate2 + (i64)b * d.gate_ld + chan, g2);
                }
                float du[KC], y[KC], dh[KC];
                unpack16<T>(rp[u], du);
                unpack16<T>(ry[u], y);
                float h[KC], sp[KC];
#pragma unroll
                for (int i = 0; i < KC; ++i) h[i] = fmaf(y[i], sc[i], sh[i]);
                silu_grad_n<KC>(h, sp);
#pragma unroll
                for (int i = 0; i < KC; ++i) dh[i] = fmaf(du[i], g[i], g2[i]) * sp[i];
                if (dh_out) st_vec<T>(dh_out + row * d.ld + chan, dh);
#pragma unroll
                for (int i = 0; i < KC; ++i) { float r = round_t<T>(dh[i]); s0[i] += r; s1[i] += r * (y[i] - m3[i]) * i3[i]; }
            }
        }
    }
    slice_stats_flush<KC>(lstat, s0, s1, cv, c0, C, stats, blockIdx.x % DWN_NREP);
    DET_EXIT();
}
int k_bn3_bwd_reduce(const LoadDesc& d, const float* coef3, i64 rows, int C, double* stats, void* dh_out, int dtype, hipStream_t s) {
    DISPATCH_T(dtype,
        hipLaunchKernelGGL((bn3_bwd_reduce_kernel<bf16_t>), resident_slice_grid(bn3_bwd_reduce_kernel<bf16_t>, rows, C, 8), dim3(256), 0, s, d, coef3, rows, C, stats, (bf16_t*)dh_out),
        hipLaunchKernelGGL((bn3_bwd_reduce_kernel<float>), resident_slice_grid(bn3_bwd_reduce_kernel<float>, rows, C, 4), dim3(256), 0, s, d, coef3, rows, C, stats, (float*)dh_out));
    DWN_CHECK_LAUNCH();
    return 0;
}

__global__ __launch_bounds__(256) void pwl_bwd_reduce_kernel(const float* __restrict__ P, const float* __restrict__ gate,
                                                             const float* __restrict__ W, int B, int K, int N,
                                                             float* __restrict__ dW, float* __restrict__ dg) {
    __shared__ float red[4][16][64 + 4];
    const int nq = threadIdx.x & 15, kl = threadIdx.x >> 4;
    const int n = blockIdx.x * 64 + nq * 4, b0 = blockIdx.y * 4;
    float dgp[4][4], gt[4][4];
#pragma unroll
    for (int bb = 0; bb < 4; ++bb)
#pragma unroll
        for (int j = 0; j < 4; ++j) { dgp[bb][j] = 0.f; gt[bb][j] = 0.f; }
    const bool vec = (N & 3) == 0 && n + 3 < N;
    const bool nok = n < N;
    DET_ENTER();
    if (nok) {
#pragma unroll
        for (int bb = 0; bb < 4; ++bb)
            if (b0 + bb < B)
#pragma unroll
                for (int j = 0; j < 4; ++j)
                    if (n + j < N) gt[bb][j] = gate[(i64)(b0 + bb) * N + n + j];
        for (int k = kl; k < K; k += 16) {
            float w[4], dwa[4] = {0.f, 0.f, 0.f, 0.f}, p[4][4];
            if (vec) {
                const float4 w4 = *reinterpret_cast<const float4*>(W + (i64)k * N + n);
                w[0] = w4.x; w[1] = w4.y; w[2] = w4.z; w[3] = w4.w;
#pragma unroll
                for (int bb = 0; bb < 4; ++bb) {
                    const int b = b0 + bb < B ? b0 + bb : B - 1;
                    const float4 p4 = *reinterpret_cast<const float4*>(P + ((i64)b * K + k) * N + n);
                    p[bb][0] = p4.x; p[bb][1] = p4.y; p[bb][2] = p4.z; p[bb][3] = p4.w;
                }
            } else {
#pragma unroll
                for (int j = 0; j < 4; ++j) w[j] = n + j < N ? W[(i64)k * N + n + j] : 0.f;
#pragma unroll
                for (int bb = 0; bb < 4; ++bb) {
                    const int b = b0 + bb < B ? b0 + bb : B - 1;
#pragma unroll
                    for (int j = 0; j < 4; ++j) p[bb][j] = n + j < N ? P[((i64)b * K + k) * N + n + j] : 0.f;
                }
            }
#pragma unroll
            for (int bb = 0; bb < 4; ++bb)
#pragma unroll
                for (int j = 0; j < 4; ++j) {
                    dgp[bb][j] = fmaf(w[j], p[bb][j], dgp[bb][j]);
                    dwa[j] = fmaf(gt[bb][j], p[bb][j], dwa[j]);
                }
#pragma unroll
            for (int j = 0; j < 4; ++j)
                if (n + j < N) atomicAdd(dW + (i64)k * N + n + j, dwa[j]);
        }
    }
#pragma unroll
    for (int bb = 0; bb < 4; ++bb)
#pragma unroll
        for (int j = 0; j < 4; ++j) red[bb][kl][nq * 4 + j] = dgp[bb][j];
    __syncthreads();
    {
        const int bb = threadIdx.x >> 6, nl = threadIdx.x & 63;
        const int nn = blockIdx.x * 64 + nl;
        if (nn < N && b0 + bb < B) {
            float t = 0.f;
#pragma unroll
            for (int q = 0; q < 16; ++q) t += red[bb][q][nl];
            dg[(i64)(b0 + bb) * N + nn] = t;
        }
    }
    DET_EXIT();
}
int k_pwl_bwd_reduce(const float* P, const float* gate, const float* W, int B, int K, int N, float* dW, float* dg,
                     hipStream_t s) {
    hipLaunchKernelGGL(pwl_bwd_reduce_kernel, dim3((N + 63) / 64, (B + 3) / 4), dim3(256), 0, s, P, gate, W, B, K, N, dW, dg);
    DWN_CHECK_LAUNCH();
    return 0;
}

template <typename T>
__global__ __launch_bounds__(256) void pool_fwd_kernel(const T* x, T* out, i64 BT, int HW, int C) {
    SLICE_SETUP(C)
// ... 822 lines not shown
            if (!q.transpose) { if (rd < q.R && cd < q.C) v = q.src[((i64)g * q.R + rd) * q.C + cd]; }
            else { if (cd < q.R && rd < q.C) v = q.src[((i64)g * q.R + cd) * q.C + rd]; }
            reinterpret_cast<T*>(q.dst)[idx] = from_f<T>(v);
        }
    }
}
int k_prep(const PrepArgs& pa, int dtype, hipStream_t s) {
    int total = 0;
    for (int i = 0; i < pa.nops; ++i) total += pa.op[i].nblocks;
    if (total == 0) return 0;
    DISPATCH_T(dtype,
        hipLaunchKernelGGL((prep_kernel<bf16_t>), dim3(total), dim3(256), 0, s, pa),
        hipLaunchKernelGGL((prep_kernel<float>), dim3(total), dim3(256), 0, s, pa));
    DWN_CHECK_LAUNCH();
    return 0;
}



template <typename T>
__global__ __launch_bounds__(256) void pw_bwd_prep_kernel(const float* w1, const float* abc, int E, int C, T* bp, float* gacc,
                                                          float* r3, int nscale, int gx, int gy, int gr) {
    const i64 ld = (i64)E + C;
    int bid = blockIdx.x;
    __shared__ float sA[64][64 + 4], sB[64][64 + 4];
    if (bid < nscale) {
        const int nkt = (E + 63) / 64;
        const int k0 = (bid % nkt) * 64, n0 = (bid / nkt) * 64;
        for (int i = threadIdx.x; i < 64 * 64; i += 256) {
            const int kl = i >> 6, nl = i & 63;
            const int k = k0 + kl, n = n0 + nl;
            sA[kl][nl] = (k < E && n < C) ? abc[k] * round_t<T>(w1[(i64)k * C + n]) : 0.f;
        }
        __syncthreads();
        for (int i = threadIdx.x; i < 64 * 64; i += 256) {
            const int nl = i >> 6, kl = i & 63;
            const int k = k0 + kl, n = n0 + nl;
            if (k < E && n < C) bp[n * ld + k] = from_f<T>(sA[kl][nl]);
        }
        DET_EXIT();
        return;
    }
    bid -= nscale;
    const int GR = gr;
    const int bx = bid % gx, by = (bid / gx) % gy, bz = bid / (gx * gy);
    const int e0 = bz * GR;
    const float* A2 = abc + E;
    const float* A3 = abc + 2 * E;
    for (int i = threadIdx.x; i < GR * 64; i += 256) {
        const int el = i >> 6, cl = i & 63;
        const int e = e0 + el;
        const int cpg = bx * 64 + cl, cg = by * 64 + cl;
        const bool eok = e < E;
        sA[el][cl] = (eok && cpg < C) ? A2[e] * round_t<T>(w1[(i64)e * C + cpg]) : 0.f;
        sB[el][cl] = (eok && cg < C) ? round_t<T>(w1[(i64)e * C + cg]) : 0.f;
    }
    __syncthreads();
    const int ty = threadIdx.x >> 4, tx = threadIdx.x & 15;
    float acc[4][4], acc3[4];
#pragma unroll
    for (int i = 0; i < 4; ++i) {
        acc3[i] = 0.f;
#pragma unroll
        for (int j = 0; j < 4; ++j) acc[i][j] = 0.f;
    }
    const bool do_r3 = bx == 0 && ty == 0;
#pragma unroll 8
    for (int el = 0; el < GR; ++el) {
        const float4 a4 = *reinterpret_cast<const float4*>(&sA[el][ty * 4]);
        const float4 b4 = *reinterpret_cast<const float4*>(&sB[el][tx * 4]);
        const float a[4] = {a4.x, a4.y, a4.z, a4.w}, b[4] = {b4.x, b4.y, b4.z, b4.w};
#pragma unroll
        for (int i = 0; i < 4; ++i)
#pragma unroll
            for (int j = 0; j < 4; ++j) acc[i][j] = fmaf(a[i], b[j], acc[i][j]);
        if (do_r3) {
            const float a3 = e0 + el < E ? A3[e0 + el] : 0.f;
#pragma unroll
            for (int j = 0; j < 4; ++j) acc3[j] = fmaf(a3, b[j], acc3[j]);
        }
    }
    DET_ENTER();
#pragma unroll
    for (int i = 0; i < 4; ++i) {
        const int cp = bx * 64 + ty * 4 + i;
#pragma unroll
        for (int j = 0; j < 4; ++j) {
            const int c = by * 64 + tx * 4 + j;
            if (cp < C && c < C) atomicAdd(gacc + (i64)cp * C + c, acc[i][j]);
        }
    }
    if (do_r3) {
#pragma unroll
        for (int j = 0; j < 4; ++j) {
            const int c = by * 64 + tx * 4 + j;
            if (c < C) atomicAdd(r3 + c, acc3[j]);
        }
    }
    DET_EXIT();
}
template <typename T>
__global__ __launch_bounds__(256) void pw_bwd_gram_store_kernel(const float* gacc, int E, int C, T* bp, const float* res_abc, int res_C,
                                                                float* r3) {
    const i64 idx = (i64)blockIdx.x * 256 + threadIdx.x;
    if (idx >= (i64)C * C) return;
    const int cp = (int)(idx / C), c = (int)(idx % C);
    float g = gacc[idx];
    if (res_abc && cp == c) {
        float d2 = 0.f, d3 = 0.f;
        for (int cc = c; cc < res_C; cc += C) { d2 += res_abc[res_C + cc]; d3 += res_abc[2 * res_C + cc]; }
        g += d2;
        r3[c] += d3;
    }
    bp[(i64)c * ((i64)E + C) + E + cp] = from_f<T>(g);
}
int k_pw_bwd_prep(const float* w1, const float* abc, int E, int C, void* bp, float* gacc, float* r3, int dtype,
                  const float* res_abc, int res_C, hipStream_t s) {
    const int nscale = ((E + 63) / 64) * ((C + 63) / 64);
    const int gr = C <= 64 ? 32 : 64;
    const int gx = (C + 63) / 64, gy = (C + 63) / 64, gz = (E + gr - 1) / gr;
    const int ngram = gx * gy * gz;
    DISPATCH_T(dtype,
        hipLaunchKernelGGL((pw_bwd_prep_kernel<bf16_t>), dim3(nscale + ngram), dim3(256), 0, s, w1, abc, E, C, (bf16_t*)bp, gacc, r3, nscale, gx, gy, gr),
        hipLaunchKernelGGL((pw_bwd_prep_kernel<float>), dim3(nscale + ngram), dim3(256), 0, s, w1, abc, E, C, (float*)bp, gacc, r3, nscale, gx, gy, gr));
    DWN_CHECK_LAUNCH();
    dim3 g3((unsigned)(((i64)C * C + 255) / 256));
    DISPATCH_T(dtype,
        hipLaunchKernelGGL((pw_bwd_gram_store_kernel<bf16_t>), g3, dim3(256), 0, s, gacc, E, C, (bf16_t*)bp, res_abc, res_C, r3),
        hipLaunchKernelGGL((pw_bwd_gram_store_kernel<float>), g3, dim3(256), 0, s, gacc, E, C, (float*)bp, res_abc, res_C, r3));
    DWN_CHECK_LAUNCH();
    return 0;
}

size_t pw_wgrad_tacc_floats(int E, int C) { return (size_t)(E + C + 8) * C; }
template <typename T>
__global__ __launch_bounds__(256) void pw_wgrad_fold_kernel(const float* __restrict__ tacc, const float* __restrict__ abc,
                                                            const float* __restrict__ w1, int E, int C, float* __restrict__ dw) {
    const i64 idx = (i64)blockIdx.x * 256 + threadIdx.x;
    if (idx >= (i64)E * C) return;
    const int e = (int)(idx / C), c = (int)(idx % C);
    const float* ga = tacc + (i64)E * C + c;
    const float* wrow = w1 + (i64)e * C;
    float g0 = 0.f, g1 = 0.f, g2 = 0.f, g3 = 0.f;
    for (int cp = 0; cp < C; cp += 4) {
        g0 = fmaf(round_t<T>(wrow[cp]), ga[(i64)cp * C], g0);
        g1 = fmaf(round_t<T>(wrow[cp + 1]), ga[(i64)(cp + 1) * C], g1);
        g2 = fmaf(round_t<T>(wrow[cp + 2]), ga[(i64)(cp + 2) * C], g2);
        g3 = fmaf(round_t<T>(wrow[cp + 3]), ga[(i64)(cp + 3) * C], g3);
    }
    const float g = (g0 + g1) + (g2 + g3);
    dw[idx] = fmaf(abc[e], tacc[idx], fmaf(abc[E + e], g, abc[2 * E + e] * tacc[(i64)(E + C) * C + c]));
}
template <typename T, int CC>
__global__ __launch_bounds__(256) void pw_wgrad_fold_tile_kernel(const float* __restrict__ tacc, const float* __restrict__ abc,
                                                                 const float* __restrict__ w1, int E, float* __restrict__ dw) {
    constexpr int G = 256 / CC, ROWS = 4 * G;
    __shared__ __attribute__((aligned(16))) float sw[CC][ROWS];
    const int tid = threadIdx.x, e0 = blockIdx.x * ROWS;
    for (int i = tid; i < ROWS * CC; i += 256) {
        const int row = i / CC, cp = i % CC;
        sw[cp][row] = e0 + row < E ? round_t<T>(w1[(i64)(e0 + row) * CC + cp]) : 0.f;
    }
    __syncthreads();
    const int c = tid % CC, gq = tid / CC;
    const float* ga = tacc + (i64)E * CC + c;
    float acc[4] = {0.f, 0.f, 0.f, 0.f};
#pragma unroll 1
    for (int cp0 = 0; cp0 < CC; cp0 += 16) {
        float gv[16];
#pragma unroll
        for (int u = 0; u < 16; ++u) gv[u] = ga[(i64)(cp0 + u) * CC];
#pragma unroll
        for (int u = 0; u < 16; ++u) {
            const float4 w4 = *reinterpret_cast<const float4*>(&sw[cp0 + u][gq * 4]);
            acc[0] = fmaf(w4.x, gv[u], acc[0]);
            acc[1] = fmaf(w4.y, gv[u], acc[1]);
            acc[2] = fmaf(w4.z, gv[u], acc[2]);
            acc[3] = fmaf(w4.w, gv[u], acc[3]);
        }
    }
    const float sc = tacc[(i64)(E + CC) * CC + c];
#pragma unroll
    for (int r = 0; r < 4; ++r) {
        const int e = e0 + gq * 4 + r;
        if (e < E) dw[(i64)e * CC + c] = fmaf(abc[e], tacc[(i64)e * CC + c], fmaf(abc[E + e], acc[r], abc[2 * E + e] * sc));
    }
}
int k_pw_wgrad_fold(const float* tacc, const float* abc, const float* w1, int E, int C, float* dw, int dtype, hipStream_t s) {
#define FOLD_TILE(CC_) do { \
        dim3 grid((unsigned)((E + 4 * (256 / CC_) - 1) / (4 * (256 / CC_)))); \
        DISPATCH_T(dtype, \
            hipLaunchKernelGGL((pw_wgrad_fold_tile_kernel<bf16_t, CC_>), grid, dim3(256), 0, s, tacc, abc, w1, E, dw), \
            hipLaunchKernelGGL((pw_wgrad_fold_tile_kernel<float, CC_>), grid, dim3(256), 0, s, tacc, abc, w1, E, dw)); \
        DWN_CHECK_LAUNCH(); \
        return 0; } while (0)
    if (C == 64) FOLD_TILE(64);
    if (C == 128) FOLD_TILE(128);
    if (C == 256) FOLD_TILE(256);
#undef FOLD_TILE
    dim3 grid((unsigned)(((i64)E * C + 255) / 256));
    DISPATCH_T(dtype,
        hipLaunchKernelGGL((pw_wgrad_fold_kernel<bf16_t>), grid, dim3(256), 0, s, tacc, abc, w1, E, C, dw),
        hipLaunchKernelGGL((pw_wgrad_fold_kernel<float>), grid, dim3(256), 0, s, tacc, abc, w1, E, C, dw));
    DWN_CHECK_LAUNCH();
    return 0;
}
```

sensorium_amd/csrc/dwn_kernels.h:

```cpp
#pragma once
#include "dwn_internal.h"

struct ResGeom {
    int BT, T, Hin, Win, Hout, Wout, Cin, Cout;
    const int* hsrc; const int* wsrc;
    const int* hinv; const int* winv;
};

typedef dwn_tensor_entry TensorListEntry;

struct BnFinJob {
    const double* stats; int stat_c; double count; const float* gamma; const float* beta;
    float* running_mean; float* running_var; long long* nbt; float* coef; int C; int nblocks;
};
struct BnBwdJob { const double* stats; double count; const float* coef; float* dgamma; float* dbeta; float* abc; int C; int nblocks; int frozen; };
int k_bn_finalize_train(BnFinJob j0, BnFinJob j1, float momentum, float eps, hipStream_t s);
int k_bn_bwd_finalize(BnBwdJob j0, BnBwdJob j1, hipStream_t s);
int k_bn_finalize_eval(const float* gamma, const float* beta, const float* rm, const float* rv, float eps,
                       float* coef, int C, hipStream_t s);
int k_bn1_gram_finalize(const double* gram, const float* w1, int E, int Cin, double count, const float* gamma, const float* beta,
                        float* rm, float* rv, long long* nbt, float momentum, float eps, float* coef, double* sc_stats, int dtype,
                        hipStream_t s);
int k_ew_apply(const LoadDesc& d, int kind, void* out, i64 ldo, i64 rows, int C, int dtype, hipStream_t s);
int k_stem_xmom(const float* x, int B, int Cin, i64 S, double* mom, hipStream_t s);
int k_stem_bn_finalize(const double* mom, double count, const float* w, const float* gamma, const float* beta, float* rm,
                       float* rv, long long* nbt, float momentum, float eps, float* coef, double* xmom, int C0, int Cin,
                       hipStream_t s);
int k_stem_out(const float* x, const float* w, const float* coef, const float* pe_t, const float* pe_h, const float* pe_w,
               int Tn, int H, int W, int B, int Cin, i64 S, int C0, void* out, int dtype, hipStream_t s);
int k_stem_bwd_acc(const void* dout, const float* x, const double* xmom, double count, int B, int Cin, i64 S, int C0,
                   double* acc, int dtype, hipStream_t s);
int k_stem_bwd_finalize(const double* acc, const double* xmom, const float* w, const float* coef, double count, float* dgamma,
                        float* dbeta, float* dw, int C0, int Cin, hipStream_t s);
int k_stem_bwd_finalize_frozen(const double* acc, const float* w, const float* coef, float* dgamma, float* dbeta, float* dw,
                               int C0, int Cin, hipStream_t s);
int k_stem_input_grad(const void* dout, const float* w, const float* coef, int B, int Cin, i64 S, int C0, float* dx, int dtype,
                      hipStream_t s);
int k_stem_bwd_finalize_dx(const double* acc, const double* xmom, const float* w, const float* coef, double count, float* qx,
                           int C0, int Cin, hipStream_t s);
int k_stem_input_grad_train(const void* dout, const float* w, const float* coef, const float* x, const float* qx, int B, int Cin,
                            i64 S, int C0, float* dx, int dtype, hipStream_t s);
int stem_moment_count();
int stem_acc_stride();
int k_shortcut_stats(const LoadDesc& xin, const ResGeom& gm, double* stats, int dtype, hipStream_t s);
int k_residual_fwd(const LoadDesc& xin, const void* y4, const float* coef4, const float* coefsc, const float* dscale,
                   const ResGeom& gm, const float* ope_t, const float* ope_h, const float* ope_w, void* out, int dtype,
                   hipStream_t s);
int k_residual_bwd_reduce(const LoadDesc& xin, const void* y4, const void* dout, const float* coef4,
                          const float* coefsc, const float* dscale, const ResGeom& gm, double* stats4,
                          double* statssc, int dtype, hipStream_t s);
int k_residual_bwd_dy4(const void* y4, const void* dout, const float* abc4, const float* dscale, const ResGeom& gm,
                       void* dy4, int dtype, hipStream_t s);
int k_residual_bwd_dx(const LoadDesc& xin, const void* da0, const void* dout, const float* abcsc, const ResGeom& gm,
                      void* dx, int dtype, hipStream_t s);
int k_se_pool(const LoadDesc& z3, int B, int C, int rows_per_sample, long long* pooled, void* z3out, int dtype, hipStream_t s);
int k_se_mlp_fwd(const long long* pooled_sum, float inv_s, const float* wr, const float* br, const float* we,
                 const float* be, int B, int C, int R, float* pmean, float* hid_pre, float* gate, const float* w2, void* wg, int N2,
                 int dtype, int* folded, hipStream_t s);
int k_se_mlp_bwd(const float* dg, const float* gate, const float* hid_pre, const float* pmean, const float* wr,
                 const float* we, int B, int C, int R, float inv_s, float* dgp, float* dhp, float* dps, float* dwr,
                 float* dbr, float* dwe, float* dbe, hipStream_t s);
int k_bn3_bwd_reduce(const LoadDesc& d, const float* coef3, i64 rows, int C, double* stats, void* dh_out, int dtype, hipStream_t s);
int k_pool_fwd(const void* x, void* out, i64 BT, int HW, int C, int dtype, hipStream_t s);
int k_pool_bwd(const void* dpool, void* dx, i64 BT, int HW, int C, int dtype, hipStream_t s);
int k_cortex_residual_fwd(const void* y, const void* x, const float* coef, const float* coefsc, const float* dscale,
                          int M, int Tn, int Cin, int C, int groups, void* out, int dtype, hipStream_t s);
int k_cortex_stats(const void* y, const void* x, int M, int Cin, int C, double* stats, double* statssc, int dtype, hipStream_t s);
int k_cortex_bwd_reduce(const void* y, const void* x, const void* dout, const float* gmask, int gmask_ld,
                        const float* coef, const float* coefsc, const float* dscale, int M, int Tn, int Cin, int C,
                        int groups, double* stats, double* statssc, int dtype, hipStream_t s);
int k_cortex_bwd_dy(const void* y, const void* dout, const float* gmask, int gmask_ld, const float* coef,
                    const float* abc, const float* dscale, int M, int Tn, int C, int groups, void* dy, int dtype,
                    hipStream_t s);
int k_cortex_bwd_dx(const void* dxmain, const void* x, const void* dout, const float* gmask, int gmask_ld,
                    const float* abcsc, int M, int Tn, int Cin, int C, void* dx, int dtype, hipStream_t s);
int k_pack_weight(const float* src, void* dst, int groups, int R, int C, int transpose, int Rd, int Cd, int dtype,
                  hipStream_t s);
int k_gate_weights(const float* w, const float* gate, void* dst, int B, int N, int K, int dtype, hipStream_t s);
size_t k_readout_dbeta_parts(int B, int Rp, int groups);
int k_readout_dz(const float* dout, const float* out, float beta, const float* beta_dev, double* part, float* dbeta, int B, int Tn, int n_valid, int Rg, int Rp,
                 int groups, void* dz, float* db, int dtype, hipStream_t s);
int k_poisson_fwd(const float* pred, const float* target, const float* w, i64 per_sample, i64 total, float eps,
                  double* loss, hipStream_t s);
int k_poisson_bwd(const float* pred, const float* target, const float* w, const float* gscale, i64 per_sample,
                  i64 total, float eps, float* dpred, hipStream_t s);
int k_f64_to_f32(const double* src, float* dst, int n, hipStream_t s);
int k_adamw_ema(const TensorListEntry* list, int ntensors, int max_blocks, float decay_w, float omb1, float beta2,
                float omb2, float eps, float step_size, float bc2_sqrt, float ema_decay, float ema_omd,
                float grad_scale, hipStream_t s);
int k_ema_lerp(const TensorListEntry* list, int ntensors, int max_blocks, float decay, float omd, hipStream_t s);
int k_grad_sumsq(const dwn_guarded_entry* list, int ntensors, int max_blocks, double grad_scale, void* ws, double* pair,
                 hipStream_t s);
int k_step_guard_finalize(const double* pair_a, const double* pair_b, double max_norm, int skip_nonfinite,
                          const dwn_guarded_entry* list, int ntensors, dwn_step_guard* guard, hipStream_t s);
int k_adamw_ema_guarded(const dwn_guarded_entry* list, int ntensors, int max_blocks, double lr, double beta1, double beta2,
                        double eps, double weight_decay, double ema_decay, double grad_scale, const dwn_step_guard* guard,
                        hipStream_t s);
int k_fill_f32(float* p, float v, int n, hipStream_t s);
int k_pack_weight_dual(const float* src, void* plain, void* tr, int groups, int R, int C, int Rp, int ldp, int ldt, int dtype,
                       hipStream_t s);
int k_pwl_bwd_reduce(const float* P, const float* gate, const float* W, int B, int K, int N, float* dW, float* dg,
                     hipStream_t s);
int k_assemble_inputs(const dwn_clip_desc* descs, int B, int T, int H0, int W0, int H, int W, float pad, float* x,
                      hipStream_t s);
int k_assemble_targets(const dwn_clip_desc* descs, int B, int T, float* const* targets, const int* n_neurons,
                       int n_mice, int max_neurons, float* mice_weights, hipStream_t s);
int k_zero(void* p, size_t nbytes, hipStream_t s);
int k_gaze_forward(const dwn_gaze_args& a, hipStream_t s);
int k_gaze_backward(const dwn_gaze_args& a, hipStream_t s);
int k_plane_mean(const float* x, int B, int Cin, int T, int H, int W, int c0, int nc, float* mean, hipStream_t s);
size_t k_corr_ws_bytes(int N);
int k_corr_moments(const dwn_corr_args& a, hipStream_t s);
int k_corr_finalize(const dwn_corr_args& a, hipStream_t s);
int k_corr_backward(const dwn_corr_args& a, hipStream_t s);

size_t k_gabor_ws_bytes(const dwn_gabor_args& a);
int k_gabor_forward(const dwn_gabor_args& a, hipStream_t s);
int k_gabor_backward(const dwn_gabor_args& a, hipStream_t s);

size_t k_blur3d_ws_bytes(const dwn_blur3d_args& a);
int k_blur3d(const dwn_blur3d_args& a, hipStream_t s);
size_t k_clip_moments_ws_bytes(const dwn_clip_moments_args& a);
int k_clip_moments(const dwn_clip_moments_args& a, hipStream_t s);
int k_mei_update(const dwn_mei_update_args& a, hipStream_t s);
size_t k_trial_score_ws_bytes(int N);
int k_trial_moments(const dwn_trial_score_args& a, hipStream_t s);
int k_trial_score_finalize(const dwn_trial_score_args& a, hipStream_t s);
size_t k_modulator_ws_bytes(const dwn_modulator_args& a);
int k_modulator_forward(const dwn_modulator_args& a, hipStream_t s);
int k_modulator_backward(const dwn_modulator_args& a, hipStream_t s);
size_t k_spatial_gain_ws_bytes(const dwn_spatial_gain_args& a);
int k_spatial_gain_forward(const dwn_spatial_gain_args& a, hipStream_t s);
int k_spatial_gain_backward(const dwn_spatial_gain_args& a, hipStream_t s);
int k_noise_forward(const dwn_noise_args& a, hipStream_t s);
size_t k_sta_state_bytes(const dwn_sta_args& a);
size_t k_sta_ws_bytes(const dwn_sta_args& a);
int k_sta_accumulate(const dwn_sta_args& a, hipStream_t s);
int k_sta_finalize(const dwn_sta_args& a, hipStream_t s);
size_t k_gauss2d_ws_bytes(const dwn_gauss2d_args& a);
int k_gauss2d_fit(const dwn_gauss2d_args& a, hipStream_t s);
int k_gauss2d_profile(const dwn_gauss2d_profile_args& a, hipStream_t s);
long long k_pair_ldz(int N);
size_t k_pair_compare_ws_bytes(int M);
int k_pair_stage(const dwn_pair_args& a, hipStream_t s);
int k_pair_syrk(const dwn_pair_args& a, hipStream_t s);
int k_pair_corr_finalize(const dwn_pair_args& a, hipStream_t s);
int k_pair_compare(const dwn_pair_compare_args& a, hipStream_t s);
int k_pw_bwd_prep(const float* w1, const float* abc, int E, int C, void* bp, float* gacc, float* r3, int dtype,
                  const float* res_abc, int res_C, hipStream_t s);
size_t pw_wgrad_tacc_floats(int E, int C);
int k_pw_wgrad_fold(const float* tacc, const float* abc, const float* w1, int E, int C, float* dw, int dtype, hipStream_t s);

enum { PREP_ZERO = 0, PREP_FILL = 1, PREP_PACKW = 2, PREP_PACKDW = 3, PREP_BNEVAL = 4 };
#define PREP_MAX_OPS 16
struct PrepOp {
    int kind, nblocks;
    const float* src; void* dst;
    const float* src2; const float* src3; const float* src4;
    long long n;
    float v;
    int R, C, transpose, Rd, Cd;
};
struct PrepArgs {
    int nops;
    PrepOp op[PREP_MAX_OPS];
    PrepArgs() : nops(0) {}
    static int blocks_for(long long n, int cap) { long long b = (n + 255) / 256; return (int)(b > cap ? cap : b); }
    bool zero(void* p, size_t nbytes) {
        if (nbytes == 0) return true;
        if (((size_t)p & 15) || (nbytes & 15) || nops >= PREP_MAX_OPS) return false;
        PrepOp& q = op[nops++]; q = PrepOp(); q.kind = PREP_ZERO; q.dst = p; q.n = (long long)(nbytes / 16); q.nblocks = blocks_for(q.n, 256);
        return true;
    }
    bool fill(float* p, float v, int n) {
        if (n <= 0) return true;
        if (nops >= PREP_MAX_OPS) return false;
        PrepOp& q = op[nops++]; q = PrepOp(); q.kind = PREP_FILL; q.dst = p; q.v = v; q.n = n; q.nblocks = blocks_for(n, 1 << 30);
        return true;
    }
    bool packw(const float* src, void* dst, int groups, int R, int C, int transpose, int Rd, int Cd) {
        if (nops >= PREP_MAX_OPS) return false;
        PrepOp& q = op[nops++]; q = PrepOp(); q.kind = PREP_PACKW; q.src = src; q.dst = dst; q.R = R; q.C = C; q.transpose = transpose;
        q.Rd = Rd; q.Cd = Cd; q.n = (long long)groups * Rd * Cd; q.nblocks = blocks_for(q.n, 1 << 30);
        return true;
    }
    bool packdw(const float* src, float* dst, int C, int taps) {
        if (nops >= PREP_MAX_OPS) return false;
        PrepOp& q = op[nops++]; q = PrepOp(); q.kind = PREP_PACKDW; q.src = src; q.dst = dst; q.C = C; q.R = taps; q.n = (long long)C * taps;
        q.nblocks = blocks_for(q.n, 1 << 30);
        return true;
    }
    bool bneval(const dwn_bn& bn, int C, float eps) {
        if (nops >= PREP_MAX_OPS) return false;
        PrepOp& q = op[nops++]; q = PrepOp(); q.kind = PREP_BNEVAL; q.src = bn.gamma; q.src2 = bn.beta; q.src3 = bn.running_mean;
        q.src4 = bn.running_var; q.dst = bn.coef; q.v = eps; q.n = C; q.C = C; q.nblocks = blocks_for(C, 1 << 30);
        return true;
    }
};
int k_prep(const PrepArgs& pa, int dtype, hipStream_t s);
```

Measured before the change: 1486.

## Add streamed bf16 MFMA Gram kernel for 64-channel BN1 stats and fuse param tail

Adds a dedicated bf16 64-channel Gram kernel. It computes only the upper-triangular tiles with MFMA and LDS transpose reads, and prefetches rows through registers. It spreads its atomic adds across 8 replica buffers, which a new specialised finalize kernel sums. Separately, the SE-MLP weight-gradient and pointwise weight-gradient fold at the end of block backward are merged into one tail kernel to save a launch. The aim is to replace the generic TN GEMM for the Gram statistics and reduce launch count and atomic contention, at the cost of a larger workspace and extra code specialised to 64-channel bf16.

After: 1508, median of 6. 1.4% higher.

```diff
diff --git a/sensorium_amd/_lib.py b/sensorium_amd/_lib.py
--- a/sensorium_amd/_lib.py
+++ b/sensorium_amd/_lib.py
@@ -424,7 +424,7 @@
 
 
 HASH_SRCS = ("dwn_api.hip", "dwn_gemm.hip", "dwn_gemm_nn_1.hip", "dwn_gemm_nn_2.hip", "dwn_gemm_nn_3.hip", "dwn_gemm_nn_4.hip", "dwn_gemm_nn_5.hip",
-             "dwn_gemm_nn_6.hip", "dwn_gemm_tn.hip", "dwn_pw_bwd.hip", "dwn_gemm_xl.hip", "dwn_gemm_kd.hip", "dwn_dwconv.hip", "dwn_dwrc.hip",
+             "dwn_gemm_nn_6.hip", "dwn_gemm_tn.hip", "dwn_gram.hip", "dwn_pw_bwd.hip", "dwn_gemm_xl.hip", "dwn_gemm_kd.hip", "dwn_dwconv.hip", "dwn_dwrc.hip",
              "dwn_dwbwd.hip", "dwn_dwfwd.hip", "dwn_elementwise.hip", "dwn_data.hip", "dwn_gaze.hip", "dwn_modulator.hip", "dwn_spatial.hip", "dwn_mei.hip", "dwn_rf_fit.hip", "dwn_pairwise.hip", "dwn_trial_score.hip", "dwn_rf.hip", "dwn_corr.hip", "dwn_stim.hip", "dwn_common.h", "dwn_internal.h",
              "dwn_kernels.h", "dwn_launch.h", "dwn_gemm_nn.h", "dwn_gain.h", "dwn_reduce.h",
              "../../include/dwn.h")
diff --git a/sensorium_amd/csrc/dwn_api.hip b/sensorium_amd/csrc/dwn_api.hip
--- a/sensorium_amd/csrc/dwn_api.hip
+++ b/sensorium_amd/csrc/dwn_api.hip
@@ -221,7 +221,7 @@
     w.st4 = c.take<double>(nstat(a.Cout));
     w.stsc = c.take<double>(nstat(backward ? a.Cout : a.Cin));
     w.pooled = c.take<long long>((size_t)a.B * a.Cmid);
-    if (!backward && block_y1_free(a)) w.gram = c.take<double>((size_t)(a.Cin + 8) * a.Cin);
+    if (!backward && block_y1_free(a)) w.gram = c.take<double>((size_t)gram_nrep(a.dtype, a.Cin) * (a.Cin + 8) * a.Cin);
     size_t z1 = c.off;
     if (backward) {
         w.abc1 = c.take<float>(3 * (size_t)a.Cmid);
@@ -365,7 +365,10 @@
     ENTER(device);
     return k_bn_bwd_finalize(bwd_job(stats, count, *bn, abc, C, false), BnBwdJob{}, (hipStream_t)stream);
 }
-size_t dwn_conv_pw_bn_stats_workspace_bytes(int Cin) { return (size_t)(Cin + 8) * Cin * sizeof(double) + 256; }
+size_t dwn_conv_pw_bn_stats_workspace_bytes(int Cin) {
+    const int nrep = gram_nrep(DWN_BF16, Cin) > gram_nrep(DWN_F32, Cin) ? gram_nrep(DWN_BF16, Cin) : gram_nrep(DWN_F32, Cin);
+    return (size_t)nrep * (Cin + 8) * Cin * sizeof(double) + 256;
+}
 int dwn_conv_pw_bn_stats(const void* a0, long long a0_ld, long long M, const float* w_pw, int E, int Cin, const dwn_bn* bn,
                          float momentum, float eps, double* sc_stats, void* ws, size_t ws_bytes, int dtype, int device, void* stream) {
     ENTER(device);
@@ -374,13 +377,18 @@
     if (Cin % 8 || E <= 0 || M <= 0 || M >= (1ll << 31)) return dwn_set_error(-2, "conv_pw_bn_stats: Cin % 8 == 0, 0 < M < 2^31");
     if (ws_bytes < dwn_conv_pw_bn_stats_workspace_bytes(Cin)) return dwn_set_error(-6, "conv_pw_bn_stats: workspace too small");
     double* gram = reinterpret_cast<double*>(((size_t)ws + 255) & ~(size_t)255);
-    TRY(k_zero(gram, (size_t)(Cin + 8) * Cin * sizeof(double), s));
-    LoadDesc cat = ld_plain(a0, a0_ld);
-    cat.cat_c1 = Cin; cat.cat_c2 = 0;
-    GemmTN g = tn_base(cat, LD_CAT1, ld_plain(a0, a0_ld), LD_PLAIN, (int)M, Cin + 8, Cin, reinterpret_cast<float*>(gram), Cin, 1);
-    g.dw_f64 = 1;
-    TRY(launch_gemm_tn(g, dtype, s));
-    return k_bn1_gram_finalize(gram, w_pw, E, Cin, (double)M, bn->gamma, bn->beta, bn->running_mean, bn->running_var,
+    const int nrep = gram_nrep(dtype, Cin);
+    TRY(k_zero(gram, (size_t)nrep * (Cin + 8) * Cin * sizeof(double), s));
+    bool streamed = false;
+    TRY(k_gram(a0, a0_ld, M, Cin, gram, dtype, &streamed, s));
+    if (!streamed) {
+        LoadDesc cat = ld_plain(a0, a0_ld);
+        cat.cat_c1 = Cin; cat.cat_c2 = 0;
+        GemmTN g = tn_base(cat, LD_CAT1, ld_plain(a0, a0_ld), LD_PLAIN, (int)M, Cin + 8, Cin, reinterpret_cast<float*>(gram), Cin, 1);
+        g.dw_f64 = 1;
+        TRY(launch_gemm_tn(g, dtype, s));
+    }
+    return k_bn1_gram_finalize(gram, streamed ? nrep : 1, w_pw, E, Cin, (double)M, bn->gamma, bn->beta, bn->running_mean, bn->running_var,
                                bn->num_batches_tracked, momentum, eps, bn->coef, sc_stats, dtype, s);
 }
 int dwn_pack_weight(const float* src, void* dst, int groups, int R, int C, int transpose, int Rd, int Cd, int dtype,
@@ -532,10 +540,14 @@
         LoadDesc cat = ld_plain(a0, a.Cin);
         cat.cat_c1 = a.Cin; cat.cat_c2 = 0;
         if (bs) {
+        bool streamed = false;
+        PROF(DWN_FAM_PW_FWD, k_gram(a0, a.Cin, Min, a.Cin, w.gram, dt, &streamed, s));
+        if (!streamed) {
         GemmTN g = tn_base(cat, LD_CAT1, ld_plain(a0, a.Cin), LD_PLAIN, (int)Min, a.Cin + 8, a.Cin, reinterpret_cast<float*>(w.gram), a.Cin, 1);
         g.dw_f64 = 1;
         PROF(DWN_FAM_PW_FWD, launch_gemm_tn(g, dt, s));
-        PROF(DWN_FAM_PW_FWD, k_bn1_gram_finalize(w.gram, a.w_pw, a.Cmid, a.Cin, (double)Min, a.bn1.gamma, a.bn1.beta, a.bn1.running_mean,
+        }
+        PROF(DWN_FAM_PW_FWD, k_bn1_gram_finalize(w.gram, streamed ? gram_nrep(dt, a.Cin) : 1, a.w_pw, a.Cmid, a.Cin, (double)Min, a.bn1.gamma, a.bn1.beta, a.bn1.running_mean,
                                                  a.bn1.running_var, a.bn1.num_batches_tracked, a.momentum, a.eps, a.bn1.coef,
                                                  identity_sc ? w.stsc : nullptr, dt, s));
         }
@@ -614,7 +626,7 @@
 
 static int pw_backward(int dt, const void* dh1, const void* a0, const float* w_pw, const float* abc, int E, int Cin, i64 M,
                        void* bp, float* gacc, float* r3, float* tacc, void* da0, float* dw, const void* res,
-                       const float* res_abc, int res_C, const ResGeom* rg, hipStream_t s) {
+                       const float* res_abc, int res_C, const ResGeom* rg, hipStream_t s, bool fold = true) {
     const int res_n = res ? res_C / Cin : 0;
     const bool gathered = res && rg && rg->hinv;
     if (res && (!res_abc || res_C % Cin || res_n < 1 || res_n > 2))
@@ -639,6 +651,7 @@
             PROF(DWN_FAM_PW_WGRAD, launch_gemm_tn(g, dt, s));
         }
     }
+    if (!fold) return 0;
     return k_pw_wgrad_fold(tacc, abc, w_pw, E, Cin, dw, dt, s);
 }
 
@@ -693,7 +706,7 @@
         }
         PROF(DWN_FAM_PWL_WGRAD, k_pwl_bwd_reduce(w.pb, a.se_gate, a.w_pwl, a.B, a.Cout, a.Cmid, a.dw_pwl, dg, s));
         TRY(k_se_mlp_bwd(dg, a.se_gate, a.se_hidpre, a.se_pmean, a.se_wr, a.se_we, a.B, a.Cmid, a.se_r,
-                         1.0f / (float)S_out, w.dgp, w.dhp, w.dps, a.dse_wr, a.dse_br, a.dse_we, a.dse_be, s));
+                         1.0f / (float)S_out, w.dgp, w.dhp, w.dps, a.dse_wr, a.dse_br, a.dse_we, a.dse_be, s, false));
         GemmNN g = nn_base(ld_plain(a.dy4, a.Cout), LD_PLAIN, w.wpwl, a.Cout, du, a.Cmid, (int)Mout, a.Cmid, a.Cout, 1);
         g.epi = EPI_DH3; g.y3 = a.y3; g.ldy3 = a.Cmid; g.gate3 = a.se_gate; g.dps3 = w.dps; g.dg_ld = a.Cmid;
         g.coef3 = a.bn3.coef; g.coef3_ld = a.Cmid; g.rows_per_sample = S_out;
@@ -713,7 +726,7 @@
         PROF(DWN_FAM_PWL_WGRAD, launch_gemm_tn(g, dt, s));
     }
     TRY(k_se_mlp_bwd(dg, a.se_gate, a.se_hidpre, a.se_pmean, a.se_wr, a.se_we, a.B, a.Cmid, a.se_r,
-                     1.0f / (float)S_out, w.dgp, w.dhp, w.dps, a.dse_wr, a.dse_br, a.dse_we, a.dse_be, s));
+                     1.0f / (float)S_out, w.dgp, w.dhp, w.dps, a.dse_wr, a.dse_br, a.dse_we, a.dse_be, s, false));
     LoadDesc d3; memset(&d3, 0, sizeof(d3));
     d3.p = du; d3.q = a.y3; d3.ld = a.Cmid; d3.v1 = w.ident3; d3.v2 = w.ident3 + a.Cmid; d3.v3 = w.ident3 + 2 * a.Cmid;
     d3.v4 = a.bn3.coef; d3.v5 = a.bn3.coef + a.Cmid; d3.gate = a.se_gate; d3.gate2 = w.dps; d3.gate_ld = a.Cmid;
@@ -746,10 +759,10 @@
     const bool dx_folded = a.Cout % a.Cin == 0 && a.Cout / a.Cin <= 2 && dwn_pw_bwd_fused_supported(dt, Min, a.Cmid, a.Cin) &&
                            (identity_sc || (gm.hinv && gm.winv && a.Hin + a.Win <= 512));
     TRY(pw_backward(dt, dh1, xin.p, a.w_pw, w.abc1, a.Cmid, a.Cin, Min, w.bp, w.gacc, w.r3, w.tacc, dx_folded ? a.dx : a.da0, a.dw_pw,
-                    dx_folded ? a.dout : nullptr, w.abcsc, a.Cout, (dx_folded && !identity_sc) ? &gm : nullptr, s));
-    if (dx_folded) return 0;
-    PROF(DWN_FAM_RESID_BWD, k_residual_bwd_dx(xin, a.da0, a.dout, w.abcsc, gm, a.dx, dt, s));
-    return 0;
+                    dx_folded ? a.dout : nullptr, w.abcsc, a.Cout, (dx_folded && !identity_sc) ? &gm : nullptr, s, false));
+    if (!dx_folded) PROF(DWN_FAM_RESID_BWD, k_residual_bwd_dx(xin, a.da0, a.dout, w.abcsc, gm, a.dx, dt, s));
+    return k_block_param_tail(w.dgp, w.dhp, a.se_pmean, a.se_hidpre, a.B, a.Cmid, a.se_r, a.dse_wr, a.dse_br, a.dse_we, a.dse_be,
+                              w.tacc, w.abc1, a.w_pw, a.Cmid, a.Cin, a.dw_pw, dt, s);
 }
 
 int dwn_block_forward_writes(const dwn_block_args* ap) {
diff --git a/sensorium_amd/csrc/dwn_elementwise.hip b/sensorium_amd/csrc/dwn_elementwise.hip
--- a/sensorium_amd/csrc/dwn_elementwise.hip
+++ b/sensorium_amd/csrc/dwn_elementwise.hip
@@ -162,6 +162,24 @@
     return 0;
 }
 
+__device__ __forceinline__ void bn1_gram_write(int e, int E, double lin, double quad, double count, const float* gamma, const float* beta,
+                                               float* running_mean, float* running_var, float momentum, float eps, float* coef) {
+    const double inv_n = 1.0 / count;
+    const double mean = lin * inv_n;
+    double var = quad * inv_n - mean * mean;
+    if (var < 0) var = 0;
+    const float invstd = (float)(1.0 / sqrt(var + (double)eps));
+    const float scale = gamma[e] * invstd;
+    coef[e] = scale;
+    coef[E + e] = beta[e] - (float)mean * scale;
+    coef[2 * E + e] = (float)mean;
+    coef[3 * E + e] = invstd;
+    if (running_mean) {
+        const double unbiased = count > 1 ? var * count / (count - 1) : var;
+        running_mean[e] = (1.f - momentum) * running_mean[e] + momentum * (float)mean;
+        running_var[e] = (1.f - momentum) * running_var[e] + momentum * (float)unbiased;
+    }
+}
 template <typename T>
 __global__ __launch_bounds__(256) void bn1_gram_finalize_kernel(const double* __restrict__ gram, const float* __restrict__ w1,
                                                                 int E, int Cin, double count, const float* gamma, const float* beta,
@@ -180,7 +198,6 @@
     if (e >= E) return;
     for (int j = lane; j < Cin; j += 64) lw[wv][j] = round_t<T>(w1[(i64)e * Cin + j]);
     __builtin_amdgcn_wave_barrier();
-    const double inv_n = 1.0 / count;
     double quad = 0.0, lin = 0.0;
     for (int i = lane; i < Cin; i += 64) {
         const double* grow = gram + (i64)i * Cin;
@@ -195,24 +212,77 @@
 #pragma unroll
     for (int o = 32; o > 0; o >>= 1) { quad += __shfl_xor(quad, o); lin += __shfl_xor(lin, o); }
     if (lane != 0) return;
-    const double mean = lin * inv_n;
-    double var = quad * inv_n - mean * mean;
-    if (var < 0) var = 0;
-    const float invstd = (float)(1.0 / sqrt(var + (double)eps));
-    const float scale = gamma[e] * invstd;
-    coef[e] = scale;
-    coef[E + e] = beta[e] - (float)mean * scale;
-    coef[2 * E + e] = (float)mean;
-    coef[3 * E + e] = invstd;
-    if (running_mean) {
-        const double unbiased = count > 1 ? var * count / (count - 1) : var;
-        running_mean[e] = (1.f - momentum) * running_mean[e] + momentum * (float)mean;
-        running_var[e] = (1.f - momentum) * running_var[e] + momentum * (float)unbiased;
-    }
-}
-int k_bn1_gram_finalize(const double* gram, const float* w1, int E, int Cin, double count, const float* gamma, const float* beta,
+    bn1_gram_write(e, E, lin, quad, count, gamma, beta, running_mean, running_var, momentum, eps, coef);
+}
+__device__ __forceinline__ int gram64_offset(int k) {
+    if (k >= 10 * 256) return 64 * 64 + (k - 10 * 256);
+    const int t = k >> 8;
+    const int bi = t < 4 ? 0 : t < 7 ? 1 : t < 9 ? 2 : 3;
+    const int bj = t - (bi == 0 ? 0 : bi == 1 ? 3 : bi == 2 ? 5 : 6);
+    return (bi * 16 + ((k >> 4) & 15)) * 64 + bj * 16 + (k & 15);
+}
+template <typename T, int NREP>
+__global__ __launch_bounds__(256) void bn1_gram64_finalize_kernel(const double* __restrict__ gram, const float* __restrict__ w1,
+                                                                  int E, double count, const float* gamma, const float* beta,
+                                                                  float* running_mean, float* running_var, long long* nbt,
+                                                                  float momentum, float eps, float* coef, double* sc_stats) {
+    constexpr int C = 64, TILE = 256, NT = 10;
+    constexpr i64 REP = (i64)(C + 8) * C;
+    __shared__ double gs[C][C];
+    __shared__ double ssum[C];
+    __shared__ float lw[4][C];
+    const int tid = threadIdx.x, lane = tid & 63, wv = tid >> 6;
+    const int e = blockIdx.x * 4 + wv;
+    if (blockIdx.x == 0 && tid == 0 && nbt) *nbt += 1;
+    constexpr int NP = (NT * TILE + C) / 2, NIT = (NP + 255) / 256;
+    double2 v[NIT][NREP];
+#pragma unroll
+    for (int it = 0; it < NIT; ++it) {
+        int p = tid + 256 * it;
+        if (p > NP - 1) p = NP - 1;
+        const double2* gp = reinterpret_cast<const double2*>(gram + gram64_offset(2 * p));
+#pragma unroll
+        for (int r = 0; r < NREP; ++r) v[it][r] = gp[r * (REP / 2)];
+    }
+#pragma unroll
+    for (int it = 0; it < NIT; ++it) {
+        const int p = tid + 256 * it, k = 2 * p;
+        double2 a = make_double2(0.0, 0.0);
+#pragma unroll
+        for (int r = 0; r < NREP; ++r) { a.x += v[it][r].x; a.y += v[it][r].y; }
+        if (p >= NP) continue;
+        if (k >= NT * TILE) { ssum[k - NT * TILE] = a.x; ssum[k - NT * TILE + 1] = a.y; continue; }
+        const int off = gram64_offset(k), i = off / C, j = off % C;
+        gs[i][j] = a.x; gs[i][j + 1] = a.y;
+        if ((i >> 4) != (j >> 4)) { gs[j][i] = a.x; gs[j + 1][i] = a.y; }
+    }
+    if (e < E) lw[wv][lane] = round_t<T>(w1[(i64)e * C + lane]);
+    __syncthreads();
+    if (sc_stats && blockIdx.x == 0 && tid < C) {
+        sc_stats[tid] = ssum[tid];
+        sc_stats[C + tid] = gs[tid][tid];
+    }
+    if (e >= E) return;
+    double r = 0.0;
+#pragma unroll 8
+    for (int j = 0; j < C; ++j) r += gs[j][lane] * (double)lw[wv][j];
+    double quad = (double)lw[wv][lane] * r, lin = (double)lw[wv][lane] * ssum[lane];
+#pragma unroll
+    for (int o = 32; o > 0; o >>= 1) { quad += __shfl_xor(quad, o); lin += __shfl_xor(lin, o); }
+    if (lane != 0) return;
+    bn1_gram_write(e, E, lin, quad, count, gamma, beta, running_mean, running_var, momentum, eps, coef);
+}
+int k_bn1_gram_finalize(const double* gram, int nrep, const float* w1, int E, int Cin, double count, const float* gamma, const float* beta,
                         float* rm, float* rv, long long* nbt, float momentum, float eps, float* coef, double* sc_stats, int dtype,
                         hipStream_t s) {
+    if (nrep > 1) {
+        if (Cin != 64 || dtype != DWN_BF16 || nrep != DWN_GRAM_NREP)
+            return dwn_set_error(-2, "bn1_gram_finalize: replicas are the bf16, 64-channel Gram kernel's (DWN_GRAM_NREP of them)");
+        hipLaunchKernelGGL((bn1_gram64_finalize_kernel<bf16_t, DWN_GRAM_NREP>), dim3((E + 3) / 4), dim3(256), 0, s, gram, w1, E, count, gamma, beta,
+                           rm, rv, nbt, momentum, eps, coef, sc_stats);
+        DWN_CHECK_LAUNCH();
+        return 0;
+    }
     if (Cin > 512 || Cin % 4) return dwn_set_error(-2, "bn1_gram_finalize: Cin must be a multiple of 4, at most 512");
     if (dtype == DWN_BF16)
         hipLaunchKernelGGL(bn1_gram_finalize_kernel<bf16_t>, dim3((E + 3) / 4), dim3(256), 0, s, gram, w1, E, Cin, count, gamma, beta,
@@ -1444,11 +1514,10 @@
     }
 }
 
-__global__ __launch_bounds__(256) void se_mlp_wgrad_kernel(const float* dgp, const float* dhp, const float* pmean,
-                                                           const float* hid_pre, int B, int C, int R, float* dwr,
-                                                           float* dbr, float* dwe, float* dbe) {
-    const int c = blockIdx.x * 256 + threadIdx.x;
-    const int r = blockIdx.y;
+__device__ __forceinline__ void se_mlp_wgrad_body(int bx, int r, const float* dgp, const float* dhp, const float* pmean,
+                                                  const float* hid_pre, int B, int C, int R, float* dwr, float* dbr, float* dwe,
+                                                  float* dbe) {
+    const int c = bx * 256 + threadIdx.x;
     if (c < C) {
         float a = 0.f, a2 = 0.f, sb = 0.f;
 #pragma unroll 8
@@ -1462,11 +1531,16 @@
         dwr[(i64)r * C + c] = a2;
         if (r == 0) dbe[c] = sb;
     }
-    if (blockIdx.x == 0 && threadIdx.x == 0) {
+    if (bx == 0 && threadIdx.x == 0) {
         float sb = 0.f;
         for (int b = 0; b < B; ++b) sb += dhp[(i64)b * R + r];
         dbr[r] = sb;
     }
+}
+__global__ __launch_bounds__(256) void se_mlp_wgrad_kernel(const float* dgp, const float* dhp, const float* pmean,
+                                                           const float* hid_pre, int B, int C, int R, float* dwr,
+                                                           float* dbr, float* dwe, float* dbe) {
+    se_mlp_wgrad_body((int)blockIdx.x, (int)blockIdx.y, dgp, dhp, pmean, hid_pre, B, C, R, dwr, dbr, dwe, dbe);
 }
 
 int k_se_mlp_fwd(const long long* pooled_sum, float inv_s, const float* wr, const float* br, const float* we,
@@ -1496,7 +1570,7 @@
 }
 int k_se_mlp_bwd(const float* dg, const float* gate, const float* hid_pre, const float* pmean, const float* wr,
                  const float* we, int B, int C, int R, float inv_s, float* dgp, float* dhp, float* dps, float* dwr,
-                 float* dbr, float* dwe, float* dbe, hipStream_t s) {
+                 float* dbr, float* dwe, float* dbe, hipStream_t s, bool wgrad) {
     if ((R & 1) == 0 && R <= SE_RT && !((size_t)we & 15)) {
 #define SE_BWD_FOLD(RP_) do { \
         if ((R & 3) == 0) hipLaunchKernelGGL((se_mlp_bwd_fold_kernel<RP_, 4>), dim3(B, 8), dim3(256), 0, s, dg, gate, hid_pre, wr, we, C, R, inv_s, dgp, dhp, dps); \
@@ -1510,6 +1584,7 @@
                            C, R, inv_s, dgp, dhp, dps);
     }
     DWN_CHECK_LAUNCH();
+    if (!wgrad) return 0;
     hipLaunchKernelGGL(se_mlp_wgrad_kernel, dim3((C + 255) / 256, R), dim3(256), 0, s, dgp, dhp, pmean, hid_pre, B, C, R,
                        dwr, dbr, dwe, dbe);
     DWN_CHECK_LAUNCH();
@@ -2638,11 +2713,11 @@
     dw[idx] = fmaf(abc[e], tacc[idx], fmaf(abc[E + e], g, abc[2 * E + e] * tacc[(i64)(E + C) * C + c]));
 }
 template <typename T, int CC>
-__global__ __launch_bounds__(256) void pw_wgrad_fold_tile_kernel(const float* __restrict__ tacc, const float* __restrict__ abc,
-                                                                 const float* __restrict__ w1, int E, float* __restrict__ dw) {
+__device__ __forceinline__ void pw_wgrad_fold_tile_body(int bx, const float* __restrict__ tacc, const float* __restrict__ abc,
+                                                        const float* __restrict__ w1, int E, float* __restrict__ dw) {
     constexpr int G = 256 / CC, ROWS = 4 * G;
     __shared__ __attribute__((aligned(16))) float sw[CC][ROWS];
-    const int tid = threadIdx.x, e0 = blockIdx.x * ROWS;
+    const int tid = threadIdx.x, e0 = bx * ROWS;
     for (int i = tid; i < ROWS * CC; i += 256) {
         const int row = i / CC, cp = i % CC;
         sw[cp][row] = e0 + row < E ? round_t<T>(w1[(i64)(e0 + row) * CC + cp]) : 0.f;
@@ -2671,6 +2746,11 @@
         const int e = e0 + gq * 4 + r;
         if (e < E) dw[(i64)e * CC + c] = fmaf(abc[e], tacc[(i64)e * CC + c], fmaf(abc[E + e], acc[r], abc[2 * E + e] * sc));
     }
+}
+template <typename T, int CC>
+__global__ __launch_bounds__(256) void pw_wgrad_fold_tile_kernel(const float* __restrict__ tacc, const float* __restrict__ abc,
+                                                                 const float* __restrict__ w1, int E, float* __restrict__ dw) {
+    pw_wgrad_fold_tile_body<T, CC>((int)blockIdx.x, tacc, abc, w1, E, dw);
 }
 int k_pw_wgrad_fold(const float* tacc, const float* abc, const float* w1, int E, int C, float* dw, int dtype, hipStream_t s) {
 #define FOLD_TILE(CC_) do { \
@@ -2691,3 +2771,38 @@
     DWN_CHECK_LAUNCH();
     return 0;
 }
+
+template <typename T, int CC>
+__global__ __launch_bounds__(256) void block_param_tail_kernel(const float* dgp, const float* dhp, const float* pmean,
+                                                               const float* hid_pre, int B, int Cse, int R, float* dwr, float* dbr,
+                                                               float* dwe, float* dbe, int gxse, int nse,
+                                                               const float* __restrict__ tacc, const float* __restrict__ abc,
+                                                               const float* __restrict__ w1, int E, float* __restrict__ dw) {
+    const int job = (int)blockIdx.x;
+    if (job < nse) {
+        se_mlp_wgrad_body(job % gxse, job / gxse, dgp, dhp, pmean, hid_pre, B, Cse, R, dwr, dbr, dwe, dbe);
+        return;
+    }
+    pw_wgrad_fold_tile_body<T, CC>(job - nse, tacc, abc, w1, E, dw);
+}
+int k_block_param_tail(const float* dgp, const float* dhp, const float* pmean, const float* hid_pre, int B, int Cse, int R,
+                       float* dwr, float* dbr, float* dwe, float* dbe, const float* tacc, const float* abc, const float* w1, int E,
+                       int C, float* dw, int dtype, hipStream_t s) {
+    const int gxse = (Cse + 255) / 256, nse = gxse * R;
+#define PARAM_TAIL(CC_) do { \
+        dim3 grid((unsigned)(nse + (E + 4 * (256 / CC_) - 1) / (4 * (256 / CC_)))); \
+        DISPATCH_T(dtype, \
+            hipLaunchKernelGGL((block_param_tail_kernel<bf16_t, CC_>), grid, dim3(256), 0, s, dgp, dhp, pmean, hid_pre, B, Cse, R, \
+                               dwr, dbr, dwe, dbe, gxse, nse, tacc, abc, w1, E, dw), \
+            hipLaunchKernelGGL((block_param_tail_kernel<float, CC_>), grid, dim3(256), 0, s, dgp, dhp, pmean, hid_pre, B, Cse, R, \
+                               dwr, dbr, dwe, dbe, gxse, nse, tacc, abc, w1, E, dw)); \
+        DWN_CHECK_LAUNCH(); \
+        return 0; } while (0)
+    if (C == 64) PARAM_TAIL(64);
+    if (C == 128) PARAM_TAIL(128);
+    if (C == 256) PARAM_TAIL(256);
+#undef PARAM_TAIL
+    hipLaunchKernelGGL(se_mlp_wgrad_kernel, dim3(gxse, R), dim3(256), 0, s, dgp, dhp, pmean, hid_pre, B, Cse, R, dwr, dbr, dwe, dbe);
+    DWN_CHECK_LAUNCH();
+    return k_pw_wgrad_fold(tacc, abc, w1, E, C, dw, dtype, s);
+}
diff --git a/sensorium_amd/csrc/dwn_gram.hip b/sensorium_amd/csrc/dwn_gram.hip
--- /dev/null
+++ b/sensorium_amd/csrc/dwn_gram.hip
@@ -0,0 +1,177 @@
+#include "dwn_gemm_nn.h"
+#include "dwn_kernels.h"
+
+#ifndef GRAM_SETS
+#define GRAM_SETS 4
+#endif
+namespace {
+constexpr int GRAM_C = 64;
+constexpr int GRAM_WAVES = 8, GRAM_THREADS = 64 * GRAM_WAVES;
+constexpr int GRAM_STEP = 32;
+constexpr int GRAM_RS = GRAM_C * 2 + 32;
+constexpr int GRAM_FOLD_GROUPS = 8 / GRAM_SETS;
+constexpr int GRAM_FOLD_ROWS = GRAM_FOLD_GROUPS * GRAM_SETS * GRAM_STEP;
+constexpr int GRAM_TILES = 10;
+constexpr int GRAM_SLOTS = 4 * GRAM_TILES + 4;
+constexpr int GRAM_MIN_STEPS = 8;
+static_assert(GRAM_FOLD_GROUPS >= 1 && GRAM_FOLD_ROWS <= 256, "fp32 partial sums cover at most 256 rows");
+static_assert(GRAM_SLOTS * 64 * (int)sizeof(double) <= GRAM_WAVES * GRAM_STEP * GRAM_RS, "the reduction image reuses the staging tiles");
+
+__device__ __forceinline__ void gram_tile_of(int t, int& bi, int& bj) {
+    bi = t < 4 ? 0 : t < 7 ? 1 : t < 9 ? 2 : 3;
+    bj = t - (bi == 0 ? 0 : bi == 1 ? 3 : bi == 2 ? 5 : 6);
+}
+
+__global__ __launch_bounds__(GRAM_THREADS) void gram64_kernel(const bf16_t* __restrict__ a0, i64 ld, i64 M, i64 steps_per_wave,
+                                                              double* __restrict__ gram, int nrep) {
+    __shared__ __attribute__((aligned(16))) unsigned char smem[GRAM_WAVES * GRAM_STEP * GRAM_RS];
+    const int tid = threadIdx.x, lane = tid & 63;
+    const int wave = __builtin_amdgcn_readfirstlane(tid >> 6);
+    const int lr = lane & 15, lg = lane >> 4;
+    unsigned char* sw = smem + wave * GRAM_STEP * GRAM_RS;
+
+    const i64 nsteps = (M + GRAM_STEP - 1) / GRAM_STEP;
+    i64 sbeg = ((i64)blockIdx.x * GRAM_WAVES + wave) * steps_per_wave;
+    i64 send = sbeg + steps_per_wave;
+    if (send > nsteps) send = nsteps;
+    if (sbeg > send) sbeg = send;
+    i64 row_end = send * GRAM_STEP;
+    if (row_end > M) row_end = M;
+
+    f32x4_t acc[GRAM_TILES], sacc[4];
+    double acc64[GRAM_TILES][4], s64[4];
+#pragma unroll
+    for (int t = 0; t < GRAM_TILES; ++t) {
+        acc[t] = f32x4_t{0.f, 0.f, 0.f, 0.f};
+#pragma unroll
+        for (int r = 0; r < 4; ++r) acc64[t][r] = 0.0;
+    }
+#pragma unroll
+    for (int b = 0; b < 4; ++b) { sacc[b] = f32x4_t{0.f, 0.f, 0.f, 0.f}; s64[b] = 0.0; }
+
+    auto fold = [&]() {
+#pragma unroll
+        for (int t = 0; t < GRAM_TILES; ++t) {
+#pragma unroll
+            for (int r = 0; r < 4; ++r) acc64[t][r] += (double)acc[t][r];
+            acc[t] = f32x4_t{0.f, 0.f, 0.f, 0.f};
+        }
+#pragma unroll
+        for (int b = 0; b < 4; ++b) { s64[b] += (double)sacc[b][0]; sacc[b] = f32x4_t{0.f, 0.f, 0.f, 0.f}; }
+    };
+
+    if (sbeg < send) {
+        const int lrow = lane >> 3, lcol = (lane & 7) * 8;
+        const i64 last = send - 1;
+        uint4 regs[GRAM_SETS][4];
+        auto issue = [&](uint4 (&r)[4], i64 s) {
+            if (s > last) s = last;
+#pragma unroll
+            for (int i = 0; i < 4; ++i) {
+                i64 row = s * GRAM_STEP + lrow + 8 * i;
+                if (row > M - 1) row = M - 1;
+                r[i] = *reinterpret_cast<const uint4*>(a0 + row * ld + lcol);
+            }
+        };
+        auto stage = [&](const uint4 (&r)[4], i64 s) {
+#pragma unroll
+            for (int i = 0; i < 4; ++i) {
+                const i64 row = s * GRAM_STEP + lrow + 8 * i;
+                const uint4 v = row < row_end ? r[i] : make_uint4(0, 0, 0, 0);
+                *reinterpret_cast<uint4*>(sw + (lrow + 8 * i) * GRAM_RS + lcol * 2) = v;
+            }
+        };
+        const bf16x8_t ones = bf16x8_t{0x3F80, 0x3F80, 0x3F80, 0x3F80, 0x3F80, 0x3F80, 0x3F80, 0x3F80};
+        auto compute = [&]() {
+            const int q = lr >> 2, p = lr & 3;
+            const int rb = 8 * lg + q;
+            bf16x8_t f[4];
+#pragma unroll
+            for (int b = 0; b < 4; ++b) {
+                const int colb = (b * 16 + 4 * p) * 2;
+                auto lo = __builtin_amdgcn_ds_read_tr16_b64_v4i16((__attribute__((address_space(3))) s16x4_t*)(sw + rb * GRAM_RS + colb));
+                auto hi = __builtin_amdgcn_ds_read_tr16_b64_v4i16((__attribute__((address_space(3))) s16x4_t*)(sw + (rb + 4) * GRAM_RS + colb));
+                f[b] = bf16x8_t{lo[0], lo[1], lo[2], lo[3], hi[0], hi[1], hi[2], hi[3]};
+            }
+            int t = 0;
+#pragma unroll
+            for (int bi = 0; bi < 4; ++bi)
+#pragma unroll
+                for (int bj = bi; bj < 4; ++bj, ++t) acc[t] = __builtin_amdgcn_mfma_f32_16x16x32_bf16(f[bi], f[bj], acc[t], 0, 0, 0);
+#pragma unroll
+            for (int b = 0; b < 4; ++b) sacc[b] = __builtin_amdgcn_mfma_f32_16x16x32_bf16(ones, f[b], sacc[b], 0, 0, 0);
+        };
+#define GRAM_LDS_ORDER() do { asm volatile("" ::: "memory"); __builtin_amdgcn_wave_barrier(); } while (0)
+#pragma unroll
+        for (int u = 0; u < GRAM_SETS; ++u) {
+            issue(regs[u], sbeg + u);
+            asm volatile("" ::: "memory");
+        }
+        int groups = 0;
+        for (i64 s = sbeg; s < send; s += GRAM_SETS) {
+#pragma unroll
+            for (int u = 0; u < GRAM_SETS; ++u) {
+                stage(regs[u], s + u);
+                GRAM_LDS_ORDER();
+                issue(regs[u], s + u + GRAM_SETS);
+                compute();
+                GRAM_LDS_ORDER();
+            }
+            if (++groups == GRAM_FOLD_GROUPS) { fold(); groups = 0; }
+        }
+        fold();
+#undef GRAM_LDS_ORDER
+    }
+
+    __syncthreads();
+    double* red = reinterpret_cast<double*>(smem);
+    for (int w = 0; w < GRAM_WAVES; ++w) {
+        if (wave == w) {
+#pragma unroll
+            for (int t = 0; t < GRAM_TILES; ++t)
+#pragma unroll
+                for (int r = 0; r < 4; ++r) {
+                    const int k = (t * 4 + r) * 64 + lane;
+                    red[k] = w == 0 ? acc64[t][r] : red[k] + acc64[t][r];
+                }
+#pragma unroll
+            for (int b = 0; b < 4; ++b) {
+                const int k = (4 * GRAM_TILES + b) * 64 + lane;
+                red[k] = w == 0 ? s64[b] : red[k] + s64[b];
+            }
+        }
+        __syncthreads();
+    }
+    DET_ENTER();
+    double* out = gram + (i64)(blockIdx.x % (unsigned)nrep) * ((GRAM_C + 8) * GRAM_C);
+    for (int k = tid; k < GRAM_SLOTS * 64; k += GRAM_THREADS) {
+        const int slot = k >> 6, l = k & 63, c = l & 15, g = l >> 4;
+        if (slot < 4 * GRAM_TILES) {
+            int bi, bj;
+            gram_tile_of(slot >> 2, bi, bj);
+            atomicAdd(out + (bi * 16 + g * 4 + (slot & 3)) * GRAM_C + bj * 16 + c, red[k]);
+        } else if (g == 0) {
+            atomicAdd(out + GRAM_C * GRAM_C + (slot - 4 * GRAM_TILES) * 16 + c, red[k]);
+        }
+    }
+    DET_EXIT();
+}
+}
+
+int gram_nrep(int dtype, int Cin) { return (dtype == DWN_BF16 && Cin == GRAM_C) ? DWN_GRAM_NREP : 1; }
+
+int k_gram(const void* a0, i64 ld, i64 M, int Cin, double* gram, int dtype, bool* done, hipStream_t s) {
+    *done = false;
+    if (gram_nrep(dtype, Cin) == 1 || M <= 0) return 0;
+    if (ld < Cin || ld % 8 || ((size_t)a0 & 15)) return dwn_set_error(-2, "gram: a0 must be 16-byte aligned with ld >= Cin a multiple of 8");
+    const i64 nsteps = (M + GRAM_STEP - 1) / GRAM_STEP;
+    const int bpc = resident_bpc(gram64_kernel, GRAM_THREADS, 0, 1);
+    const i64 grid = resident_grid_x(bpc > 1 ? 1 : bpc, 1, (nsteps + GRAM_WAVES * GRAM_MIN_STEPS - 1) / (GRAM_WAVES * GRAM_MIN_STEPS));
+    const i64 waves = grid * GRAM_WAVES;
+    const i64 steps_per_wave = (nsteps + waves - 1) / waves;
+    hipLaunchKernelGGL(gram64_kernel, dim3((unsigned)grid), dim3(GRAM_THREADS), 0, s, reinterpret_cast<const bf16_t*>(a0), ld, M,
+                       steps_per_wave, gram, DWN_GRAM_NREP);
+    DWN_CHECK_LAUNCH();
+    *done = true;
+    return 0;
+}
diff --git a/sensorium_amd/csrc/dwn_kernels.h b/sensorium_amd/csrc/dwn_kernels.h
--- a/sensorium_amd/csrc/dwn_kernels.h
+++ b/sensorium_amd/csrc/dwn_kernels.h
@@ -18,9 +18,12 @@
 int k_bn_bwd_finalize(BnBwdJob j0, BnBwdJob j1, hipStream_t s);
 int k_bn_finalize_eval(const float* gamma, const float* beta, const float* rm, const float* rv, float eps,
                        float* coef, int C, hipStream_t s);
-int k_bn1_gram_finalize(const double* gram, const float* w1, int E, int Cin, double count, const float* gamma, const float* beta,
+int k_bn1_gram_finalize(const double* gram, int nrep, const float* w1, int E, int Cin, double count, const float* gamma, const float* beta,
                         float* rm, float* rv, long long* nbt, float momentum, float eps, float* coef, double* sc_stats, int dtype,
                         hipStream_t s);
+#define DWN_GRAM_NREP 8
+int gram_nrep(int dtype, int Cin);
+int k_gram(const void* a0, i64 ld, i64 M, int Cin, double* gram, int dtype, bool* done, hipStream_t s);
 int k_ew_apply(const LoadDesc& d, int kind, void* out, i64 ldo, i64 rows, int C, int dtype, hipStream_t s);
 int k_stem_xmom(const float* x, int B, int Cin, i64 S, double* mom, hipStream_t s);
 int k_stem_bn_finalize(const double* mom, double count, const float* w, const float* gamma, const float* beta, float* rm,
@@ -59,7 +62,7 @@
                  int dtype, int* folded, hipStream_t s);
 int k_se_mlp_bwd(const float* dg, const float* gate, const float* hid_pre, const float* pmean, const float* wr,
                  const float* we, int B, int C, int R, float inv_s, float* dgp, float* dhp, float* dps, float* dwr,
-                 float* dbr, float* dwe, float* dbe, hipStream_t s);
+                 float* dbr, float* dwe, float* dbe, hipStream_t s, bool wgrad = true);
 int k_bn3_bwd_reduce(const LoadDesc& d, const float* coef3, i64 rows, int C, double* stats, void* dh_out, int dtype, hipStream_t s);
 int k_pool_fwd(const void* x, void* out, i64 BT, int HW, int C, int dtype, hipStream_t s);
 int k_pool_bwd(const void* dpool, void* dx, i64 BT, int HW, int C, int dtype, hipStream_t s);
@@ -150,6 +153,9 @@
                   const float* res_abc, int res_C, hipStream_t s);
 size_t pw_wgrad_tacc_floats(int E, int C);
 int k_pw_wgrad_fold(const float* tacc, const float* abc, const float* w1, int E, int C, float* dw, int dtype, hipStream_t s);
+int k_block_param_tail(const float* dgp, const float* dhp, const float* pmean, const float* hid_pre, int B, int Cse, int R,
+                       float* dwr, float* dbr, float* dwe, float* dbe, const float* tacc, const float* abc, const float* w1, int E,
+                       int C, float* dw, int dtype, hipStream_t s);
 
 enum { PREP_ZERO = 0, PREP_FILL = 1, PREP_PACKW = 2, PREP_PACKDW = 3, PREP_BNEVAL = 4 };
 #define PREP_MAX_OPS 16
```
